# MLAB-project/radio-observer

Measured on AMD Instinct MI355X. Metric: FFT rows/sec (spectra/sec), N=32768 75% overlap, incl. per-row bolid scan, higher is better.
Workload: dtype f32; 1 GPU; C3/C4: synthetic IQ 48 kHz, FFT bins=32768, overlap=24576 (75%), Nuttall window, waterfall magnitude rows + BolidRecorder scan; input=float32 I/Q resident in HBM, output=float32 rows in HBM, parallelism=time-chunk per GPU

## Files before the change

### include/ro_stft.h

```cpp
#ifndef RO_STFT_H
#define RO_STFT_H

#include <stddef.h>
#include <stdint.h>

#ifdef __cplusplus
extern "C" {
#endif

#define RO_OK               0
#define RO_ERR_INVALID     (-1)
#define RO_ERR_UNSUPPORTED (-2)
#define RO_ERR_HIP         (-3)
#define RO_ERR_NOMEM       (-4)
#define RO_ERR_STATE       (-5)

#define RO_ABI_VERSION 5

enum { RO_WINDOW_NUTTALL = 0, RO_WINDOW_HANN = 1, RO_WINDOW_CUSTOM = 2 };

enum { RO_IQ_F32 = 0, RO_IQ_I16 = 1, RO_IQ_F64 = 2 };

enum { RO_PRECISION_F32 = 0, RO_PRECISION_F64 = 1 };

// ... 305 lines not shown
                               ro_unit_summary_t *d_unit_summary, void *stream);

int ro_snapshot_units_host(const ro_snapshot_t *dir, int64_t dir_capacity, const ro_snap_summary_t *snap_summary,
                           const float *arena, int64_t arena_floats, int32_t cols, const ro_band_window_t *slot_windows,
                           ro_fits_unit_t *unit_dir, void *units, int64_t units_bytes, ro_unit_summary_t *unit_summary);
int ro_raw_units_host(const ro_raw_capture_t *raw_dir, int64_t dir_capacity, const ro_raw_summary_t *raw_summary,
                      const float *arena, int64_t arena_floats,
                      ro_fits_unit_t *unit_dir, void *units, int64_t units_bytes, ro_unit_summary_t *unit_summary);

#define RO_MAX_PERIODIC 8
enum { RO_PERIODIC_WRITTEN = 0, RO_PERIODIC_LOST = 1, RO_PERIODIC_NO_ROOM = 2 };

typedef struct ro_periodic {
    int32_t          snapshot_rows;
    ro_band_window_t window;
} ro_periodic_t;

typedef struct ro_periodic_entry {
    int64_t index;
    int64_t first_row;
    int64_t due_row;
    int64_t offset;
    int64_t bytes;
    int32_t rows;
    int32_t naxis1;
    int32_t recorder;
    int32_t status;
} ro_periodic_entry_t;

typedef struct ro_periodic_summary {
    int64_t entries, written, lost, no_room;
    int64_t unlisted;
    int64_t units_bytes;
    int64_t needed_bytes;
    int64_t reserved;
} ro_periodic_summary_t;

int ro_snapshot_rows(int sample_rate, int bins, int overlap, int snapshot_length);

int ro_periodic_plan(const ro_periodic_t *recorders, int count, int64_t *next_index, int64_t head_row, int final,
                     int64_t ring_rows, int32_t cols, int64_t units_bytes,
                     ro_periodic_entry_t *dir, int64_t capacity, ro_periodic_summary_t *summary);

int ro_stft_periodic_units_resident(ro_stft_t *h, const ro_row_ring_t *ring, const ro_periodic_t *recorders, int count,
                                    const ro_periodic_entry_t *dir, int64_t entries, void *d_units, int64_t units_bytes,
                                    void *stream);

int ro_periodic_units_host(const ro_row_ring_t *ring, const ro_periodic_t *recorders, int count,
                           const ro_periodic_entry_t *dir, int64_t entries, void *units, int64_t units_bytes);

#define RO_LEVEL_BLOCK 720

typedef struct ro_level_range {
    float ln_min, ln_max;
} ro_level_range_t;

int ro_stft_snapshot_levels_resident(ro_stft_t *h, const ro_snapshot_t *d_dir, int64_t dir_capacity,
                                     const ro_snap_summary_t *d_snap_summary, const float *d_arena, int64_t arena_floats,
                                     int32_t cols, const ro_band_window_t *slot_windows,
                                     ro_fits_unit_t *d_level_dir, ro_level_range_t *d_ranges, void *d_levels,
                                     int64_t levels_bytes, ro_unit_summary_t *d_level_summary, void *stream);

int ro_stft_periodic_levels_resident(ro_stft_t *h, const ro_row_ring_t *ring, const ro_periodic_t *recorders, int count,
                                     const ro_periodic_entry_t *dir, int64_t entries, ro_level_range_t *d_ranges,
                                     void *d_levels, int64_t levels_bytes, void *stream);

int ro_snapshot_levels_host(const ro_snapshot_t *dir, int64_t dir_capacity, const ro_snap_summary_t *snap_summary,
                            const float *arena, int64_t arena_floats, int32_t cols, const ro_band_window_t *slot_windows,
                            ro_fits_unit_t *level_dir, ro_level_range_t *ranges, void *levels, int64_t levels_bytes,
                            ro_unit_summary_t *level_summary);
int ro_periodic_levels_host(const ro_row_ring_t *ring, const ro_periodic_t *recorders, int count,
                            const ro_periodic_entry_t *dir, int64_t entries, ro_level_range_t *ranges, void *levels,
                            int64_t levels_bytes);

#define RO_PNG_ALIGN 16

int64_t ro_png_bytes(int32_t naxis1, int64_t naxis2);

int ro_stft_levels_png_resident(ro_stft_t *h, const ro_fits_unit_t *d_level_dir, int64_t dir_capacity,
                                const ro_unit_summary_t *d_level_summary, const void *d_levels, int64_t levels_bytes,
                                ro_fits_unit_t *d_png_dir, void *d_png, int64_t png_bytes,
                                ro_unit_summary_t *d_png_summary, void *stream);

int ro_levels_png_host(const ro_fits_unit_t *level_dir, int64_t dir_capacity, const ro_unit_summary_t *level_summary,
                       const void *levels, int64_t levels_bytes, ro_fits_unit_t *png_dir, void *png, int64_t png_bytes,
                       ro_unit_summary_t *png_summary);

int ro_stft_levels_png_deflate_resident(ro_stft_t *h, const ro_fits_unit_t *d_level_dir, int64_t dir_capacity,
                                        const ro_unit_summary_t *d_level_summary, const void *d_levels, int64_t levels_bytes,
                                        ro_fits_unit_t *d_png_dir, void *d_png, int64_t png_bytes,
                                        ro_unit_summary_t *d_png_summary, void *stream);

int ro_levels_png_deflate_host(const ro_fits_unit_t *level_dir, int64_t dir_capacity, const ro_unit_summary_t *level_summary,
                               const void *levels, int64_t levels_bytes, ro_fits_unit_t *png_dir, void *png, int64_t png_bytes,
                               ro_unit_summary_t *png_summary);

int ro_periodic_level_dir(const ro_periodic_entry_t *dir, int64_t entries, ro_fits_unit_t *level_dir,
                          ro_unit_summary_t *level_summary);

typedef struct ro_resize_info {
    int64_t jobs;
    int64_t h_items, v_items;
    int64_t mid_bytes;
    int64_t plan_bytes;
    int64_t reserved[3];
} ro_resize_info_t;

int ro_resize_shape(int32_t naxis1, int64_t naxis2, int32_t width, int32_t *out_naxis1, int64_t *out_naxis2);

int ro_resize_plan(const ro_fits_unit_t *level_dir, int64_t dir_capacity, const ro_unit_summary_t *level_summary,
                   int64_t levels_bytes, int32_t width, ro_fits_unit_t *out_level_dir, int64_t out_levels_bytes,
                   ro_unit_summary_t *out_level_summary, void *plan, int64_t plan_bytes, ro_resize_info_t *info);

int ro_stft_levels_resize_resident(ro_stft_t *h, const ro_resize_info_t *info, const void *d_plan, const void *d_levels,
                                   int64_t levels_bytes, void *d_out_levels, int64_t out_levels_bytes, void *stream);

int ro_levels_resize_host(const ro_resize_info_t *info, const void *plan, const void *levels, int64_t levels_bytes,
                          void *out_levels, int64_t out_levels_bytes);

int ro_stft_time_resident(ro_stft_t *h, const void *d_iq, int format, int64_t samples,
                          int64_t first_row, int64_t rows,
                          float *d_rows, int64_t row_stride,
                          float *d_tile, ro_scan_record_t *d_records, void *stream,
                          int iters, float *ms_out, float *kernel_ms_out);

int ro_stft_push(ro_stft_t *h, const void *iq, int format, int64_t samples, int64_t *rows_ready);
int ro_stft_flush(ro_stft_t *h, int64_t *rows_ready);
int ro_stft_fetch(ro_stft_t *h, int64_t max_rows, int first_col, int cols,
                  float *rows_out, ro_scan_record_t *records_out,
                  int64_t *first_row_index, int64_t *rows_got);
int ro_stft_fetch_sets(ro_stft_t *h, int64_t max_rows, int first_col, int cols, float *rows_out,
                       ro_scan_record_t *records_out, ro_scan_record_t *extra_out,
                       int64_t *first_row_index, int64_t *rows_got);
int ro_stft_set_tile_windows(ro_stft_t *h, const ro_band_window_t *windows, int count);
int ro_stft_tile_windows(const ro_stft_t *h, ro_band_window_t *out );
int ro_stft_rows_complete(ro_stft_t *h, int64_t *rows);
int ro_stft_set_row_sink(ro_stft_t *h, float *base, int64_t row_stride, int64_t capacity_rows, int64_t first_slot);
void *ro_pinned_alloc(int device, size_t bytes);
void  ro_pinned_free(void *p);
int   ro_pinned_check(const void *p, size_t bytes);
int ro_stft_fetch_ln(ro_stft_t *h, int64_t max_rows, float *tile_out, float *ln_out, float *minmax_out,
                     ro_scan_record_t *records_out, int64_t *first_row_index, int64_t *rows_got);
int ro_stft_reset(ro_stft_t *h);
typedef struct ro_stft_timing {
    int64_t push_calls;  double push_ms_avg, push_ms_max;
    int64_t batches;     double batch_gpu_ms_avg, batch_gpu_ms_max;
    int64_t batch_rows;  double row_gpu_us_avg;
    int64_t fetch_calls; double fetch_ms_avg, fetch_ms_max;
} ro_stft_timing_t;
int ro_stft_timing(ro_stft_t *h, ro_stft_timing_t *out, int reset );
int ro_stft_stats(const ro_stft_t *h, int64_t *samples_in, int64_t *rows_out,
                  int64_t *launches, double *kernel_ms_total);

#ifdef __cplusplus
}
#endif
#endif
```

### radio-observer_amd/__init__.py

```python
from . import build as _build
from . import capi
from .capi import (
    Stft, StftError, Bands, BandWindow, ScanRecord, PinnedArray, library, library_path, hip_runtimes, require_one_hip_runtime,
    clamp_overlap, fft_sample_rate, frequency_to_bin, bin_to_frequency, time_to_fft_samples,
    row_count, window_table, bins_supported, device_count, shard_rows, shard_samples, shard_max_rows,
    stitch_rows, ln_levels, band_supported, bands_hull, band_windows_supported, bands_windows,
    tile_windows_supported, merge_windows, events_host, Detector,
    EVENT_DTYPE, DETECT_STATE_DTYPE, DETECT_SUMMARY_DTYPE,
    snapshots_host, RowRing, ROW_RING, SNAPSHOT_DTYPE, SNAP_SUMMARY_DTYPE, RO_SNAP_CAPTURED, RO_SNAP_EMPTY, RO_SNAP_LOST,
    raw_host, IqSpan, RAW_CAPTURE_DTYPE, RAW_SUMMARY_DTYPE, RO_MAX_IQ_SPANS,
    snapshot_units_host, raw_units_host, FITS_UNIT_DTYPE, UNIT_SUMMARY_DTYPE, RO_FITS_BLOCK,
    RO_UNIT_WRITTEN, RO_UNIT_SKIPPED, RO_UNIT_NO_ROOM, RO_UNIT_INVALID,
    snapshot_rows, periodic_plan, periodic_units_host, periodic_recorders, PERIODIC_DTYPE, PERIODIC_ENTRY_DTYPE,
    PERIODIC_SUMMARY_DTYPE, RO_MAX_PERIODIC, RO_PERIODIC_WRITTEN, RO_PERIODIC_LOST, RO_PERIODIC_NO_ROOM,
    snapshot_levels_host, periodic_levels_host, LEVEL_RANGE_DTYPE, RO_LEVEL_BLOCK,
    png_bytes, levels_png_host, levels_png_deflate_host, periodic_level_dir, RO_PNG_ALIGN,
    resize_shape, resize_plan, levels_resize_host, RESIZE_INFO_DTYPE,
    RO_WINDOW_NUTTALL, RO_WINDOW_HANN, RO_WINDOW_CUSTOM, RO_IQ_F32, RO_IQ_I16, RO_IQ_F64,
    RO_PRECISION_F32, RO_PRECISION_F64,
)

def sharding():
    import importlib
    return importlib.import_module(__name__ + ".timeshard")


__all__ = ["capi", "Stft", "StftError", "Bands", "ScanRecord", "library"]
```

### radio-observer_amd/build.py

```python
import os
import subprocess
import sys

HERE = os.path.dirname(os.path.abspath(__file__))
CSRC = os.path.join(HERE, "csrc")
LIB = os.path.join(HERE, "libro_stft.so")
SOURCES = ["ro_kernels.hip", "ro_stft32k.hip", "ro_fourstep.hip", "ro_f64reg.hip", "ro_band.hip", "ro_band_f64.hip", "ro_band_windows.hip", "ro_band_windows_f64.hip", "ro_scan_sets.hip", "ro_cut_windows.hip", "ro_events.hip", "ro_snapshots.hip", "ro_raw.hip", "ro_units.hip", "ro_periodic.hip", "ro_levels.hip", "ro_png.hip", "ro_png_deflate.hip", "ro_resize.hip", "ro_stft_capi.cpp", "ro_abi_helpers.cpp",
           "ro_exchange.cpp", "ro_stream.cpp", "ro_czt.cpp", "ro_snapshots.cpp", "ro_raw.cpp", "ro_units.cpp", "ro_periodic.cpp", "ro_levels.cpp", "ro_png.cpp", "ro_png_deflate.cpp", "ro_resize.cpp"]
HEADERS = ["ro_kernels.h", "ro_band.h", "ro_band_f64.h", "ro_band_windows.h", "ro_events.h", "ro_snapshots.h", "ro_raw.h", "ro_units.h", "ro_periodic.h", "ro_levels.h", "ro_png.h", "ro_png_deflate.h", "ro_resize.h", "ro_png_crc_device.h", "ro_pack_plan.h", "ro_host.h", "ro_owned.h", "ro_fft_device.h", "ro_fft_planar.h", "ro_k32_lds.h", "ro_device_util.h", "ro_f64_device.h", "ro_narrow.h", os.path.join("..", "..", "include", "ro_stft.h")]

HIPCC_FLAGS = ["-O3", "--offload-arch=gfx950", "-std=c++17", "-fno-slp-vectorize", "-fPIC", "-shared",
               "-Wall", "-Wno-unused-function", "-Wno-inline-asm"]


def _stale():
    if not os.path.exists(LIB):
        return True
    t = os.path.getmtime(LIB)
    deps = [os.path.join(CSRC, s) for s in SOURCES + HEADERS] + [os.path.abspath(__file__)]
    return any(os.path.getmtime(d) > t for d in deps)


def build(force=False, verbose=False):
    if not force and not _stale():
        return LIB
    hipcc = os.environ.get("HIPCC", "hipcc")
    cmd = [hipcc] + HIPCC_FLAGS + ["-o", LIB] + [os.path.join(CSRC, s) for s in SOURCES]
    if verbose:
        print(" ".join(cmd), file=sys.stderr)
    subprocess.check_call(cmd)
    return LIB


if __name__ == "__main__":
    build(force="--force" in sys.argv, verbose=True)
    print(LIB)
```

### radio-observer_amd/capi.py

```python
import ctypes as C
import os

import numpy as np

from . import build as _build

RO_WINDOW_NUTTALL, RO_WINDOW_HANN, RO_WINDOW_CUSTOM = 0, 1, 2
RO_IQ_F32, RO_IQ_I16, RO_IQ_F64 = 0, 1, 2
RO_PRECISION_F32, RO_PRECISION_F64 = 0, 1
RO_MAX_EXTRA_BANDS = 7
RO_MAX_BAND_WINDOWS = 8
RO_MAX_TILE_WINDOWS = 8

RO_OK = 0
_ERR_NAMES = {-1: "RO_ERR_INVALID", -2: "RO_ERR_UNSUPPORTED", -3: "RO_ERR_HIP", -4: "RO_ERR_NOMEM",
              -5: "RO_ERR_STATE"}


class StftError(RuntimeError):
    def __init__(self, code, text):
        super().__init__("%s (%d): %s" % (_ERR_NAMES.get(code, "RO_ERR"), code, text))
        self.code = code


class Bands(C.Structure):
    _fields_ = [("low_noise", C.c_int32), ("noise_width", C.c_int32), ("low_detect", C.c_int32),
                ("detect_width", C.c_int32), ("avg_bins", C.c_int32)]


class BandWindow(C.Structure):
    _fields_ = [("first_col", C.c_int32), ("cols", C.c_int32)]

    def __iter__(self):
        return iter((self.first_col, self.cols))

    def __repr__(self):
        return "BandWindow(%d, %d)" % (self.first_col, self.cols)


class ScanRecord(C.Structure):
    _fields_ = [("noise", C.c_float), ("peak", C.c_int32), ("average", C.c_float)]


class Timing(C.Structure):
    _fields_ = [("push_calls", C.c_int64), ("push_ms_avg", C.c_double), ("push_ms_max", C.c_double),
                ("batches", C.c_int64), ("batch_gpu_ms_avg", C.c_double), ("batch_gpu_ms_max", C.c_double),
                ("batch_rows", C.c_int64), ("row_gpu_us_avg", C.c_double),
                ("fetch_calls", C.c_int64), ("fetch_ms_avg", C.c_double), ("fetch_ms_max", C.c_double)]


SCAN_DTYPE = np.dtype([("noise", np.float32), ("peak", np.int32), ("average", np.float32)])


class Detector(C.Structure):
    _fields_ = [("advance", C.c_int32), ("jitter", C.c_int32)]


EVENT_DTYPE = np.dtype([("fire_row", np.int64), ("start_row", np.int64), ("length", np.int64), ("noise", np.float32),
                        ("peak", np.int32), ("magnitude", np.float32), ("reserved", np.int32)])
DETECT_STATE_DTYPE = np.dtype([("first_detect_row", np.int64), ("last_detect_row", np.int64), ("noise", np.float32),
                               ("peak", np.int32), ("magnitude", np.float32), ("open", np.int32)])
DETECT_SUMMARY_DTYPE = np.dtype([("events", np.int64), ("detect_rows", np.int64), ("marginal_rows", np.int64)])

RO_SNAP_CAPTURED, RO_SNAP_EMPTY, RO_SNAP_LOST = 0, 1, 2


class RowRing(C.Structure):
    _fields_ = [("d_rows", C.c_void_p), ("stride", C.c_int64), ("ring_rows", C.c_int64), ("cols", C.c_int32),
                ("reserved", C.c_int32)]


ROW_RING = RowRing
SNAPSHOT_DTYPE = np.dtype([("event", EVENT_DTYPE), ("first_row", np.int64), ("offset", np.int64), ("rows", np.int32),
                           ("slot", np.int32), ("status", np.int32), ("reserved", np.int32)])
SNAP_SUMMARY_DTYPE = np.dtype([("resolved", np.int64), ("captured", np.int64), ("empty", np.int64), ("lost", np.int64),
                               ("pending", np.int64), ("pending_dropped", np.int64), ("unlisted", np.int64),
                               ("arena_floats", np.int64)])


RO_MAX_IQ_SPANS = 4


class IqSpan(C.Structure):
    _fields_ = [("d_iq", C.c_void_p), ("first_sample", C.c_int64), ("samples", C.c_int64), ("format", C.c_int32),
                ("reserved", C.c_int32)]


RAW_CAPTURE_DTYPE = np.dtype([("event", EVENT_DTYPE), ("first_sample", np.int64), ("samples", np.int64), ("offset", np.int64),
                              ("slot", np.int32), ("status", np.int32)])
RAW_SUMMARY_DTYPE = np.dtype([("resolved", np.int64), ("captured", np.int64), ("empty", np.int64), ("lost", np.int64),
                              ("pending", np.int64), ("pending_dropped", np.int64), ("arena_floats", np.int64),
                              ("reserved", np.int64)])

RO_FITS_BLOCK = 2880
RO_UNIT_WRITTEN, RO_UNIT_SKIPPED, RO_UNIT_NO_ROOM, RO_UNIT_INVALID = 0, 1, 2, 3
FITS_UNIT_DTYPE = np.dtype([("offset", np.int64), ("bytes", np.int64), ("naxis2", np.int64), ("naxis1", np.int32),
                            ("status", np.int32)])
UNIT_SUMMARY_DTYPE = np.dtype([("entries", np.int64), ("written", np.int64), ("skipped", np.int64), ("no_room", np.int64),
                               ("invalid", np.int64), ("units_bytes", np.int64), ("needed_bytes", np.int64),
                               ("reserved", np.int64)])

RO_MAX_PERIODIC = 8
RO_PERIODIC_WRITTEN, RO_PERIODIC_LOST, RO_PERIODIC_NO_ROOM = 0, 1, 2
PERIODIC_DTYPE = np.dtype([("snapshot_rows", np.int32), ("first_col", np.int32), ("cols", np.int32)])
PERIODIC_ENTRY_DTYPE = np.dtype([("index", np.int64), ("first_row", np.int64), ("due_row", np.int64), ("offset", np.int64),
                                 ("bytes", np.int64), ("rows", np.int32), ("naxis1", np.int32), ("recorder", np.int32),
                                 ("status", np.int32)])
PERIODIC_SUMMARY_DTYPE = np.dtype([("entries", np.int64), ("written", np.int64), ("lost", np.int64), ("no_room", np.int64),
                                   ("unlisted", np.int64), ("units_bytes", np.int64), ("needed_bytes", np.int64),
                                   ("reserved", np.int64)])

RO_LEVEL_BLOCK = 720
LEVEL_RANGE_DTYPE = np.dtype([("ln_min", np.float32), ("ln_max", np.float32)])
RESIZE_INFO_DTYPE = np.dtype([("jobs", np.int64), ("h_items", np.int64), ("v_items", np.int64), ("mid_bytes", np.int64),
                              ("plan_bytes", np.int64), ("reserved", np.int64, (3,))])


class Config(C.Structure):
    _fields_ = [("struct_size", C.c_uint32), ("bins", C.c_int32), ("overlap", C.c_int32),
                ("sample_rate", C.c_int32), ("window_kind", C.c_int32),
                ("window_table", C.POINTER(C.c_float)), ("iq_gain", C.c_double),
                ("iq_phase_shift", C.c_int32), ("device", C.c_int32), ("max_batch_rows", C.c_int32),
                ("enable_scan", C.c_int32), ("bands", Bands), ("tile_first_col", C.c_int32),
                ("tile_cols", C.c_int32), ("spare_cus_per_xcd", C.c_int32), ("precision", C.c_int32),
                ("tile_ln", C.c_int32)]


_EXPORTS = {
    "ro_abi_version": (C.c_int, []),
    "ro_last_error": (C.c_char_p, []),
    "ro_device_count": (C.c_int, []),
    "ro_clamp_overlap": (C.c_int, [C.c_int, C.c_int]),
    "ro_fft_sample_rate": (C.c_float, [C.c_int, C.c_int, C.c_int]),
    "ro_frequency_to_bin": (C.c_int, [C.c_int, C.c_int, C.c_float]),
    "ro_bin_to_frequency": (C.c_float, [C.c_int, C.c_int, C.c_int]),
    "ro_time_to_fft_samples": (C.c_int, [C.c_double, C.c_float]),
    "ro_row_count": (C.c_int64, [C.c_int64, C.c_int, C.c_int]),
    "ro_window_table": (C.c_int, [C.c_int, C.c_int, C.POINTER(C.c_float)]),
    "ro_bins_supported": (C.c_int, [C.c_int]),
    "ro_shard_rows": (C.c_int, [C.c_int64, C.c_int, C.c_int, C.POINTER(C.c_int64), C.POINTER(C.c_int64)]),
    "ro_shard_samples": (C.c_int, [C.c_int64, C.c_int64, C.c_int, C.c_int, C.POINTER(C.c_int64),
                                   C.POINTER(C.c_int64)]),
    "ro_shard_max_rows": (C.c_int64, [C.c_int64, C.c_int]),
    "ro_stitch_rows": (C.c_int, [C.c_void_p, C.c_int64, C.c_int, C.c_size_t, C.c_void_p]),
    "ro_direct_schedule": (C.c_int, [C.c_int, C.c_int, C.c_int64, C.c_int, C.POINTER(C.c_int), C.POINTER(C.c_int),
                                     C.POINTER(C.c_int64), C.POINTER(C.c_int64)]),
    "ro_allgather_rows": (C.c_int, [C.c_void_p, C.c_void_p, C.c_int64, C.c_int64, C.c_int, C.c_int, C.c_size_t,
                                    C.c_void_p, C.c_void_p, C.c_void_p]),
    "ro_gather_rows": (C.c_int, [C.c_void_p, C.c_void_p, C.c_int64, C.c_int64, C.c_int, C.c_int, C.c_int, C.c_size_t,
                                 C.c_void_p, C.c_void_p]),
    "ro_allgather_rows_direct": (C.c_int, [C.c_void_p, C.c_void_p, C.c_int64, C.c_int64, C.c_int, C.c_int, C.c_size_t,
                                           C.c_void_p, C.c_void_p]),
    "ro_stitch_rows_device": (C.c_int, [C.c_void_p, C.c_int64, C.c_int, C.c_size_t, C.c_void_p, C.c_void_p]),
    "ro_stft_create": (C.c_int, [C.POINTER(Config), C.POINTER(C.c_void_p)]),
    "ro_stft_destroy": (C.c_int, [C.c_void_p]),
    "ro_stft_get_window": (C.c_int, [C.c_void_p, C.POINTER(C.c_float)]),
    "ro_stft_hop": (C.c_int, [C.c_void_p]),
    "ro_stft_bins": (C.c_int, [C.c_void_p]),
    "ro_stft_device_name": (C.c_int, [C.c_void_p, C.c_char_p, C.c_size_t]),
    "ro_stft_set_bands": (C.c_int, [C.c_void_p, C.POINTER(Bands)]),
    "ro_stft_set_extra_bands": (C.c_int, [C.c_void_p, C.POINTER(Bands), C.c_int]),
    "ro_stft_extra_bands": (C.c_int, [C.c_void_p, C.POINTER(Bands)]),
    "ro_stft_run_resident_sets": (C.c_int, [C.c_void_p, C.c_void_p, C.c_int, C.c_int64, C.c_int64, C.c_int64,
                                            C.c_void_p, C.c_int64, C.c_void_p, C.c_void_p, C.c_void_p, C.c_void_p]),
    "ro_stft_scan_sets_resident": (C.c_int, [C.c_void_p, C.c_void_p, C.c_int64, C.c_int64, C.c_void_p, C.c_void_p,
                                             C.c_void_p]),
    "ro_stft_fetch_sets": (C.c_int, [C.c_void_p, C.c_int64, C.c_int, C.c_int, C.POINTER(C.c_float),
                                     C.POINTER(ScanRecord), C.POINTER(ScanRecord), C.POINTER(C.c_int64),
                                     C.POINTER(C.c_int64)]),
    "ro_stft_run_resident": (C.c_int, [C.c_void_p, C.c_void_p, C.c_int, C.c_int64, C.c_int64, C.c_int64,
                                       C.c_void_p, C.c_int64, C.c_void_p, C.c_void_p, C.c_void_p]),
    "ro_stft_run_resident_ln": (C.c_int, [C.c_void_p, C.c_void_p, C.c_int, C.c_int64, C.c_int64, C.c_int64,
                                          C.c_void_p, C.c_int64, C.c_void_p, C.c_void_p, C.c_void_p, C.c_void_p,
                                          C.c_void_p]),
    "ro_ln_levels": (C.c_int, [C.c_void_p, C.c_int64, C.c_float, C.c_float, C.c_void_p]),
    "ro_stft_fetch_ln": (C.c_int, [C.c_void_p, C.c_int64, C.c_void_p, C.c_void_p, C.c_void_p, C.c_void_p,
                                   C.POINTER(C.c_int64), C.POINTER(C.c_int64)]),
    "ro_stft_spectra_resident": (C.c_int, [C.c_void_p, C.c_void_p, C.c_int, C.c_int64, C.c_int64, C.c_int64,
                                           C.c_void_p, C.c_int64, C.c_void_p]),
    "ro_stft_scan_resident": (C.c_int, [C.c_void_p, C.c_void_p, C.c_int64, C.c_int64, C.c_void_p,
                                        C.c_void_p]),
    "ro_stft_ln_tile_resident": (C.c_int, [C.c_void_p, C.c_void_p, C.c_int64, C.c_int64, C.c_int, C.c_int,
                                           C.c_void_p, C.c_void_p, C.c_void_p, C.c_void_p]),
    "ro_stft_band_supported": (C.c_int, [C.c_int, C.c_int]),
    "ro_stft_band_supported_precision": (C.c_int, [C.c_int, C.c_int, C.c_int]),
    "ro_bands_hull": (C.c_int, [C.POINTER(Bands), C.c_int, C.c_int, C.c_int, C.POINTER(C.c_int), C.POINTER(C.c_int)]),
    "ro_stft_band_resident": (C.c_int, [C.c_void_p, C.c_void_p, C.c_int, C.c_int64, C.c_int64, C.c_int64, C.c_int,
                                        C.c_int, C.c_void_p, C.c_int64, C.c_void_p, C.c_void_p]),
    "ro_stft_band_windows_supported": (C.c_int, [C.c_int, C.POINTER(BandWindow), C.c_int, C.c_int]),
    "ro_bands_windows": (C.c_int, [C.POINTER(Bands), C.c_int, C.c_int, C.c_int, C.c_int, C.POINTER(BandWindow),
                                   C.POINTER(C.c_int)]),
    "ro_stft_band_windows_resident": (C.c_int, [C.c_void_p, C.c_void_p, C.c_int, C.c_int64, C.c_int64, C.c_int64,
                                                C.POINTER(BandWindow), C.c_int, C.c_void_p, C.c_int64, C.c_void_p,
                                                C.c_void_p, C.c_void_p]),
    "ro_tile_windows_supported": (C.c_int, [C.c_int, C.POINTER(BandWindow), C.c_int]),
    "ro_merge_windows": (C.c_int, [C.POINTER(BandWindow), C.c_int, C.c_int, C.POINTER(BandWindow), C.POINTER(C.c_int),
                                   C.POINTER(C.c_int32)]),
    "ro_stft_cut_windows_resident": (C.c_int, [C.c_void_p, C.c_void_p, C.c_int64, C.c_int64, C.POINTER(BandWindow),
                                               C.c_int, C.c_void_p, C.c_int64, C.c_void_p]),
    "ro_stft_run_resident_windows": (C.c_int, [C.c_void_p, C.c_void_p, C.c_int, C.c_int64, C.c_int64, C.c_int64,
                                               C.c_void_p, C.c_int64, C.POINTER(BandWindow), C.c_int, C.c_void_p,
                                               C.c_int64, C.c_void_p, C.c_void_p, C.c_void_p]),
    "ro_stft_set_tile_windows": (C.c_int, [C.c_void_p, C.POINTER(BandWindow), C.c_int]),
    "ro_stft_tile_windows": (C.c_int, [C.c_void_p, C.POINTER(BandWindow)]),
    "ro_events_host": (C.c_int, [C.c_void_p, C.c_int64, C.c_int64, C.c_int64, C.POINTER(Detector), C.c_void_p, C.c_void_p,
                                 C.c_int64, C.c_void_p, C.c_void_p]),
    "ro_stft_events_resident": (C.c_int, [C.c_void_p, C.c_void_p, C.c_void_p, C.c_int64, C.c_int64, C.POINTER(Detector),
                                          C.c_void_p, C.c_void_p, C.c_int64, C.c_void_p, C.c_void_p, C.c_void_p]),
    "ro_stft_run_resident_events": (C.c_int, [C.c_void_p, C.c_void_p, C.c_int, C.c_int64, C.c_int64, C.c_int64, C.c_void_p,
                                              C.c_int64, C.c_void_p, C.c_void_p, C.c_void_p, C.POINTER(Detector),
                                              C.c_void_p, C.c_void_p, C.c_int64, C.c_void_p, C.c_void_p, C.c_void_p]),
    "ro_stft_ring_put_resident": (C.c_int, [C.c_void_p, C.c_void_p, C.c_int64, C.c_int64, C.c_int64, C.POINTER(RowRing),
                                            C.c_void_p]),
    "ro_stft_snapshots_resident": (C.c_int, [C.c_void_p, C.c_void_p, C.c_int64, C.c_void_p, C.c_uint32, C.POINTER(C.c_int32),
                                             C.POINTER(RowRing), C.c_int64, C.c_void_p, C.c_void_p, C.c_int64, C.c_void_p,
                                             C.c_void_p, C.c_int64, C.c_void_p, C.c_void_p]),
    "ro_snapshots_host": (C.c_int, [C.c_void_p, C.c_int64, C.c_void_p, C.c_uint32, C.POINTER(C.c_int32), C.POINTER(RowRing),
                                    C.c_int64, C.c_void_p, C.c_void_p, C.c_int64, C.c_void_p, C.c_void_p, C.c_int64,
                                    C.c_void_p]),
    "ro_stft_raw_resident": (C.c_int, [C.c_void_p, C.c_void_p, C.c_int64, C.c_void_p, C.POINTER(IqSpan), C.c_int, C.c_void_p,
                                       C.c_void_p, C.c_int64, C.c_void_p, C.c_void_p, C.c_int64, C.c_void_p, C.c_void_p]),
    "ro_raw_host": (C.c_int, [C.c_int, C.c_int, C.c_int, C.c_void_p, C.c_int64, C.c_void_p, C.POINTER(IqSpan), C.c_int,
                              C.c_void_p, C.c_void_p, C.c_int64, C.c_void_p, C.c_void_p, C.c_int64, C.c_void_p]),
    "ro_stft_snapshot_units_resident": (C.c_int, [C.c_void_p, C.c_void_p, C.c_int64, C.c_void_p, C.c_void_p, C.c_int64, C.c_int32,
                                                  C.POINTER(BandWindow), C.c_void_p, C.c_void_p, C.c_int64, C.c_void_p,
                                                  C.c_void_p]),
    "ro_stft_raw_units_resident": (C.c_int, [C.c_void_p, C.c_void_p, C.c_int64, C.c_void_p, C.c_void_p, C.c_int64, C.c_void_p,
                                             C.c_void_p, C.c_int64, C.c_void_p, C.c_void_p]),
    "ro_snapshot_units_host": (C.c_int, [C.c_void_p, C.c_int64, C.c_void_p, C.c_void_p, C.c_int64, C.c_int32,
                                         C.POINTER(BandWindow), C.c_void_p, C.c_void_p, C.c_int64, C.c_void_p]),
    "ro_raw_units_host": (C.c_int, [C.c_void_p, C.c_int64, C.c_void_p, C.c_void_p, C.c_int64, C.c_void_p, C.c_void_p, C.c_int64,
                                    C.c_void_p]),
    "ro_snapshot_rows": (C.c_int, [C.c_int, C.c_int, C.c_int, C.c_int]),
    "ro_periodic_plan": (C.c_int, [C.c_void_p, C.c_int, C.c_void_p, C.c_int64, C.c_int, C.c_int64, C.c_int32, C.c_int64,
                                   C.c_void_p, C.c_int64, C.c_void_p]),
    "ro_stft_periodic_units_resident": (C.c_int, [C.c_void_p, C.POINTER(RowRing), C.c_void_p, C.c_int, C.c_void_p, C.c_int64,
                                                  C.c_void_p, C.c_int64, C.c_void_p]),
    "ro_periodic_units_host": (C.c_int, [C.POINTER(RowRing), C.c_void_p, C.c_int, C.c_void_p, C.c_int64, C.c_void_p, C.c_int64]),
    "ro_stft_snapshot_levels_resident": (C.c_int, [C.c_void_p, C.c_void_p, C.c_int64, C.c_void_p, C.c_void_p, C.c_int64, C.c_int32,
                                                   C.POINTER(BandWindow), C.c_void_p, C.c_void_p, C.c_void_p, C.c_int64,
                                                   C.c_void_p, C.c_void_p]),
    "ro_snapshot_levels_host": (C.c_int, [C.c_void_p, C.c_int64, C.c_void_p, C.c_void_p, C.c_int64, C.c_int32,
                                          C.POINTER(BandWindow), C.c_void_p, C.c_void_p, C.c_void_p, C.c_int64, C.c_void_p]),
    "ro_stft_periodic_levels_resident": (C.c_int, [C.c_void_p, C.POINTER(RowRing), C.c_void_p, C.c_int, C.c_void_p, C.c_int64,
                                                   C.c_void_p, C.c_void_p, C.c_int64, C.c_void_p]),
    "ro_periodic_levels_host": (C.c_int, [C.POINTER(RowRing), C.c_void_p, C.c_int, C.c_void_p, C.c_int64, C.c_void_p, C.c_void_p,
                                          C.c_int64]),
    "ro_png_bytes": (C.c_int64, [C.c_int32, C.c_int64]),
    "ro_stft_levels_png_resident": (C.c_int, [C.c_void_p, C.c_void_p, C.c_int64, C.c_void_p, C.c_void_p, C.c_int64, C.c_void_p,
                                              C.c_void_p, C.c_int64, C.c_void_p, C.c_void_p]),
    "ro_levels_png_host": (C.c_int, [C.c_void_p, C.c_int64, C.c_void_p, C.c_void_p, C.c_int64, C.c_void_p, C.c_void_p, C.c_int64,
                                     C.c_void_p]),
    "ro_stft_levels_png_deflate_resident": (C.c_int, [C.c_void_p, C.c_void_p, C.c_int64, C.c_void_p, C.c_void_p, C.c_int64,
                                                      C.c_void_p, C.c_void_p, C.c_int64, C.c_void_p, C.c_void_p]),
    "ro_levels_png_deflate_host": (C.c_int, [C.c_void_p, C.c_int64, C.c_void_p, C.c_void_p, C.c_int64, C.c_void_p, C.c_void_p,
                                             C.c_int64, C.c_void_p]),
    "ro_periodic_level_dir": (C.c_int, [C.c_void_p, C.c_int64, C.c_void_p, C.c_void_p]),
    "ro_resize_shape": (C.c_int, [C.c_int32, C.c_int64, C.c_int32, C.POINTER(C.c_int32), C.POINTER(C.c_int64)]),
    "ro_resize_plan": (C.c_int, [C.c_void_p, C.c_int64, C.c_void_p, C.c_int64, C.c_int32, C.c_void_p, C.c_int64, C.c_void_p,
                                 C.c_void_p, C.c_int64, C.c_void_p]),
    "ro_stft_levels_resize_resident": (C.c_int, [C.c_void_p, C.c_void_p, C.c_void_p, C.c_void_p, C.c_int64, C.c_void_p, C.c_int64,
                                                 C.c_void_p]),
    "ro_levels_resize_host": (C.c_int, [C.c_void_p, C.c_void_p, C.c_void_p, C.c_int64, C.c_void_p, C.c_int64]),
    "ro_stft_time_resident": (C.c_int, [C.c_void_p, C.c_void_p, C.c_int, C.c_int64, C.c_int64, C.c_int64,
                                        C.c_void_p, C.c_int64, C.c_void_p, C.c_void_p, C.c_void_p,
                                        C.c_int, C.POINTER(C.c_float), C.POINTER(C.c_float)]),
    "ro_stft_push": (C.c_int, [C.c_void_p, C.c_void_p, C.c_int, C.c_int64, C.POINTER(C.c_int64)]),
    "ro_stft_flush": (C.c_int, [C.c_void_p, C.POINTER(C.c_int64)]),
    "ro_stft_fetch": (C.c_int, [C.c_void_p, C.c_int64, C.c_int, C.c_int, C.POINTER(C.c_float),
                                C.POINTER(ScanRecord), C.POINTER(C.c_int64), C.POINTER(C.c_int64)]),
    "ro_stft_reset": (C.c_int, [C.c_void_p]),
    "ro_stft_rows_complete": (C.c_int, [C.c_void_p, C.POINTER(C.c_int64)]),
    "ro_stft_set_row_sink": (C.c_int, [C.c_void_p, C.c_void_p, C.c_int64, C.c_int64, C.c_int64]),
    "ro_pinned_alloc": (C.c_void_p, [C.c_int, C.c_size_t]),
    "ro_pinned_free": (None, [C.c_void_p]),
    "ro_pinned_check": (C.c_int, [C.c_void_p, C.c_size_t]),
    "ro_stft_timing": (C.c_int, [C.c_void_p, C.c_void_p, C.c_int]),
    "ro_stft_stats": (C.c_int, [C.c_void_p, C.POINTER(C.c_int64), C.POINTER(C.c_int64),
                                C.POINTER(C.c_int64), C.POINTER(C.c_double)]),
}

_lib = None


def library_path():
    return _build.LIB


def exported_symbols():
    return sorted(_EXPORTS)


def hip_runtimes():
    found = set()
    try:
        with open("/proc/self/maps") as f:
            for line in f:
                path = line.rsplit(None, 1)[-1]
                if "libamdhip64" in os.path.basename(path):
                    found.add(os.path.realpath(path))
    except OSError:
        pass
    return sorted(found)


def require_one_hip_runtime():
    rts = hip_runtimes()
    if len(rts) > 1:
        raise StftError(-5, "two HIP runtimes are mapped into this process (%s): import torch BEFORE radio-observer_amd "
                            "loads libro_stft.so, so that both use the same one" % ", ".join(rts))


def library():
    global _lib
    if _lib is not None:
        return _lib
    path = os.environ.get("RO_STFT_LIB")
    if not path:
        path = _build.LIB
        if not os.path.exists(path):
            _build.build()
    lib = C.CDLL(path)
    for name, (res, args) in _EXPORTS.items():
        fn = getattr(lib, name)
        fn.restype = res
        fn.argtypes = args
    _lib = lib
    return lib


class PinnedArray:

    def __init__(self, rows, cols, device=0):
        n = rows * cols * 4
        self._p = library().ro_pinned_alloc(device, n)
        if not self._p:
            raise MemoryError("ro_pinned_alloc(%d bytes) failed" % n)
        self.array = np.ctypeslib.as_array((C.c_float * (rows * cols)).from_address(self._p)).reshape(rows, cols)

    def close(self):
        if self._p:
            self.array = None
            library().ro_pinned_free(self._p)
            self._p = None

    def __del__(self):
        try:
            self.close()
        except Exception:
            pass


def _check(rc):
    if rc != RO_OK:
        raise StftError(rc, (library().ro_last_error() or b"").decode("utf-8", "replace"))


def clamp_overlap(bins, overlap):
    return library().ro_clamp_overlap(bins, overlap)


def fft_sample_rate(sample_rate, bins, overlap):
    return library().ro_fft_sample_rate(sample_rate, bins, overlap)


def frequency_to_bin(bins, sample_rate, frequency):
    return library().ro_frequency_to_bin(bins, sample_rate, frequency)


def bin_to_frequency(bins, sample_rate, bin_):
    return library().ro_bin_to_frequency(bins, sample_rate, bin_)


def time_to_fft_samples(seconds, fft_rate):
    return library().ro_time_to_fft_samples(seconds, fft_rate)


def row_count(samples, bins, overlap):
    return int(library().ro_row_count(int(samples), bins, overlap))


def window_table(kind, bins):
    w = np.empty(bins, dtype=np.float32)
    _check(library().ro_window_table(kind, bins, w.ctypes.data_as(C.POINTER(C.c_float))))
    return w


def shard_rows(total_rows, world, rank):
    first, rows = C.c_int64(), C.c_int64()
    _check(library().ro_shard_rows(int(total_rows), world, rank, C.byref(first), C.byref(rows)))
    return first.value, rows.value


def shard_samples(first_row, rows, bins, overlap):
    s0, ns = C.c_int64(), C.c_int64()
    _check(library().ro_shard_samples(int(first_row), int(rows), bins, overlap, C.byref(s0), C.byref(ns)))
    return s0.value, ns.value


def shard_max_rows(total_rows, world):
    n = library().ro_shard_max_rows(int(total_rows), world)
    if n < 0:
        _check(int(n))
    return int(n)


def direct_schedule(world, rank, total_rows, k):
    to, frm = C.c_int(), C.c_int()
    f, n = C.c_int64(), C.c_int64()
    _check(library().ro_direct_schedule(world, rank, int(total_rows), k, C.byref(to), C.byref(frm), C.byref(f), C.byref(n)))
    return to.value, frm.value, f.value, n.value


def stitch_rows(gathered, total_rows, world):
    g = np.ascontiguousarray(gathered)
    row_bytes = g.strides[0]
    out = np.empty((int(total_rows),) + g.shape[1:], dtype=g.dtype)
    _check(library().ro_stitch_rows(C.c_void_p(g.ctypes.data), int(total_rows), world, row_bytes,
                                    C.c_void_p(out.ctypes.data)))
    return out


def ln_levels(ln, mn, mx):
    a = np.ascontiguousarray(ln, dtype=np.float32)
    out = np.empty(a.shape, np.uint8)
    _check(library().ro_ln_levels(C.c_void_p(a.ctypes.data), a.size, float(mn), float(mx), C.c_void_p(out.ctypes.data)))
    return out


def bins_supported(bins):
    return bool(library().ro_bins_supported(bins))

# ... 189 lines not shown

def periodic_plan(recorders, next_index, head_row, final, ring_rows, cols, units_bytes, capacity):
    recs = periodic_recorders(recorders)
    if not isinstance(next_index, np.ndarray) or next_index.dtype != np.int64 or next_index.ndim != 1 or \
            next_index.shape[0] < len(recs) or not next_index.flags.c_contiguous:
        raise ValueError("next_index: a C-contiguous int64 array [count]")
    directory = np.zeros(max(capacity, 1), PERIODIC_ENTRY_DTYPE)
    out = np.zeros(1, PERIODIC_SUMMARY_DTYPE)
    p = lambda a: C.c_void_p(a.ctypes.data)
    _check(library().ro_periodic_plan(p(recs) if len(recs) else None, len(recs), p(next_index), head_row, 1 if final else 0,
                                      ring_rows, cols, units_bytes, p(directory) if capacity > 0 else None, capacity, p(out)))
    return directory[:int(out["entries"][0])], out[0]


def periodic_units_host(ring, recorders, directory, units_bytes, cols=None):
    ring = np.asarray(ring)
    if ring.dtype != np.float32 or ring.ndim != 2 or not ring.flags.c_contiguous:
        raise ValueError("ring: a C-contiguous float32 array [ring_rows, stride]")
    desc = RowRing(ring.ctypes.data, ring.shape[1], ring.shape[0], ring.shape[1] if cols is None else cols, 0)
    recs = periodic_recorders(recorders)
    directory = np.ascontiguousarray(directory)
    if directory.dtype != PERIODIC_ENTRY_DTYPE or directory.ndim != 1:
        raise ValueError("directory: PERIODIC_ENTRY_DTYPE [entries]")
    units = np.zeros(max(units_bytes, 1), np.uint8)
    p = lambda a: C.c_void_p(a.ctypes.data)
    _check(library().ro_periodic_units_host(C.byref(desc), p(recs) if len(recs) else None, len(recs),
                                            p(directory) if len(directory) else None, len(directory),
                                            p(units) if units_bytes > 0 else None, units_bytes))
    written = directory[directory["status"] == RO_PERIODIC_WRITTEN]
    used = 0 if not len(written) else int(written[-1]["offset"]) + -(-int(written[-1]["bytes"]) // RO_FITS_BLOCK) * RO_FITS_BLOCK
    return units[:used]


def snapshot_levels_host(directory, snap_summary, arena, cols, slot_windows, levels_bytes):
    directory = np.ascontiguousarray(directory)
    if directory.dtype != SNAPSHOT_DTYPE or directory.ndim != 1 or snap_summary.itemsize != 64 or snap_summary.size < 1:
        raise ValueError("directory: SNAPSHOT_DTYPE [n] with the summary of the call that wrote them")
    arena = np.ascontiguousarray(arena)
    if arena.dtype != np.float32 or arena.ndim != 1:
        raise ValueError("arena: float32 [arena_floats]")
    dcap = directory.shape[0]
    level_dir = np.zeros(max(dcap, 1), FITS_UNIT_DTYPE)
    ranges = np.zeros(max(dcap, 1), LEVEL_RANGE_DTYPE)
    levels = np.zeros(max(levels_bytes, 1), np.uint8)
    out = np.zeros(1, UNIT_SUMMARY_DTYPE)
    p = lambda a: C.c_void_p(a.ctypes.data)
    _check(library().ro_snapshot_levels_host(p(directory) if dcap else None, dcap, p(snap_summary), p(arena) if arena.size else None,
                                             arena.size, cols, _slot_windows(slot_windows), p(level_dir), p(ranges),
                                             p(levels) if levels_bytes > 0 else None, levels_bytes, p(out)))
    n = int(out["entries"][0])
    return level_dir[:n], ranges[:n], levels[:int(out["units_bytes"][0])], out[0]


def periodic_levels_host(ring, recorders, directory, levels_bytes, cols=None):
    ring = np.asarray(ring)
    if ring.dtype != np.float32 or ring.ndim != 2 or not ring.flags.c_contiguous:
        raise ValueError("ring: a C-contiguous float32 array [ring_rows, stride]")
    desc = RowRing(ring.ctypes.data, ring.shape[1], ring.shape[0], ring.shape[1] if cols is None else cols, 0)
    recs = periodic_recorders(recorders)
    directory = np.ascontiguousarray(directory)
    if directory.dtype != PERIODIC_ENTRY_DTYPE or directory.ndim != 1:
        raise ValueError("directory: PERIODIC_ENTRY_DTYPE [entries]")
    ranges = np.zeros(max(len(directory), 1), LEVEL_RANGE_DTYPE)
    levels = np.zeros(max(levels_bytes, 1), np.uint8)
    p = lambda a: C.c_void_p(a.ctypes.data)
    _check(library().ro_periodic_levels_host(C.byref(desc), p(recs) if len(recs) else None, len(recs),
                                             p(directory) if len(directory) else None, len(directory), p(ranges),
                                             p(levels) if levels_bytes > 0 else None, levels_bytes))
    written = directory[directory["status"] == RO_PERIODIC_WRITTEN]
    used = 0 if not len(written) else (int(written[-1]["offset"]) + -(-int(written[-1]["bytes"]) // RO_FITS_BLOCK) * RO_FITS_BLOCK) // 4
    return ranges[:len(directory)], levels[:used]


RO_PNG_ALIGN = 16


def png_bytes(naxis1, naxis2):
    n = int(library().ro_png_bytes(int(naxis1), int(naxis2)))
    if n < 0:
        _check(n)
    return n


def _levels_png_host(call, level_dir, level_summary, levels, png_room, dir_capacity):
    level_dir = np.ascontiguousarray(level_dir)
    level_summary = np.ascontiguousarray(level_summary).reshape(-1)
    if level_dir.dtype != FITS_UNIT_DTYPE or level_dir.ndim != 1 or level_summary.dtype != UNIT_SUMMARY_DTYPE or level_summary.size < 1:
        raise ValueError("level_dir: FITS_UNIT_DTYPE [n] with the UNIT_SUMMARY_DTYPE of the call that wrote them")
    levels = np.ascontiguousarray(levels)
    if levels.dtype != np.uint8 or levels.ndim != 1:
        raise ValueError("levels: uint8 [levels_bytes]")
    dcap = level_dir.shape[0] if dir_capacity is None else dir_capacity
    png_dir = np.zeros(max(dcap, 1), FITS_UNIT_DTYPE)
    png = np.zeros(max(png_room, 1), np.uint8)
    out = np.zeros(1, UNIT_SUMMARY_DTYPE)
    p = lambda a: C.c_void_p(a.ctypes.data)
    _check(call(p(level_dir) if dcap else None, dcap, p(level_summary), p(levels) if levels.size else None,
                levels.size, p(png_dir), p(png) if png_room > 0 else None, png_room, p(out)))
    return png_dir[:int(out["entries"][0])], png[:int(out["units_bytes"][0])], out[0]


def levels_png_host(level_dir, level_summary, levels, png_room, dir_capacity=None):
    return _levels_png_host(library().ro_levels_png_host, level_dir, level_summary, levels, png_room, dir_capacity)


def levels_png_deflate_host(level_dir, level_summary, levels, png_room, dir_capacity=None):
    return _levels_png_host(library().ro_levels_png_deflate_host, level_dir, level_summary, levels, png_room, dir_capacity)


def periodic_level_dir(directory):
    directory = np.ascontiguousarray(directory)
    if directory.dtype != PERIODIC_ENTRY_DTYPE or directory.ndim != 1:
        raise ValueError("directory: PERIODIC_ENTRY_DTYPE [entries]")
    level_dir = np.zeros(max(len(directory), 1), FITS_UNIT_DTYPE)
    out = np.zeros(1, UNIT_SUMMARY_DTYPE)
    p = lambda a: C.c_void_p(a.ctypes.data)
    _check(library().ro_periodic_level_dir(p(directory) if len(directory) else None, len(directory), p(level_dir), p(out)))
    return level_dir[:len(directory)], out[0]


def resize_shape(naxis1, naxis2, width):
    w, h = C.c_int32(), C.c_int64()
    _check(library().ro_resize_shape(int(naxis1), int(naxis2), int(width), C.byref(w), C.byref(h)))
    return w.value, h.value


def resize_plan(level_dir, level_summary, levels_bytes, width, out_levels_bytes, dir_capacity=None):
    level_dir = np.ascontiguousarray(level_dir)
    level_summary = np.ascontiguousarray(level_summary).reshape(-1)
    if level_dir.dtype != FITS_UNIT_DTYPE or level_dir.ndim != 1 or level_summary.dtype != UNIT_SUMMARY_DTYPE or level_summary.size < 1:
        raise ValueError("level_dir: FITS_UNIT_DTYPE [n] with the UNIT_SUMMARY_DTYPE of the call that wrote them")
    dcap = level_dir.shape[0] if dir_capacity is None else dir_capacity
    out_dir = np.zeros(max(dcap, 1), FITS_UNIT_DTYPE)
    out = np.zeros(1, UNIT_SUMMARY_DTYPE)
    info = np.zeros(1, RESIZE_INFO_DTYPE)
    p = lambda a: C.c_void_p(a.ctypes.data)
    args = (p(level_dir) if dcap else None, dcap, p(level_summary), int(levels_bytes), int(width), p(out_dir), int(out_levels_bytes), p(out))
    _check(library().ro_resize_plan(*args, None, 0, p(info)))
    plan = np.zeros(int(info["plan_bytes"][0]) // 8, np.int64).view(np.uint8)
    _check(library().ro_resize_plan(*args, p(plan), plan.size, p(info)))
    return out_dir[:int(out["entries"][0])], out[0], plan, info


def levels_resize_host(info, plan, levels, out_levels_bytes):
    info = np.ascontiguousarray(info).reshape(-1)
    plan, levels = np.ascontiguousarray(plan), np.ascontiguousarray(levels)
    if info.dtype != RESIZE_INFO_DTYPE or info.size < 1 or plan.dtype != np.uint8 or levels.dtype != np.uint8 or levels.ndim != 1:
        raise ValueError("info: RESIZE_INFO_DTYPE; plan, levels: uint8")
    out = np.zeros(max(out_levels_bytes, 1), np.uint8)
    p = lambda a: C.c_void_p(a.ctypes.data)
    _check(library().ro_levels_resize_host(p(info), p(plan), p(levels) if levels.size else None, levels.size,
                                           p(out) if out_levels_bytes > 0 else None, out_levels_bytes))
    return out[:out_levels_bytes]


def device_count():
    n = library().ro_device_count()
    if n < 0:
        _check(n)
    return n


def _ptr(x):
    if x is None:
        return None
    if hasattr(x, "data_ptr"):
        return C.c_void_p(x.data_ptr())
    return C.c_void_p(int(x))


class Stft:

    def __init__(self, bins=32768, overlap=0, sample_rate=48000, window=RO_WINDOW_NUTTALL,
                 window_table=None, iq_gain=0.0, iq_phase_shift=0, device=0, max_batch_rows=0,
                 bands=None, tile=None, spare_cus_per_xcd=0, precision=RO_PRECISION_F32, tile_ln=False,
                 extra_bands=None):
        cfg = Config()
        cfg.struct_size = C.sizeof(Config)
        cfg.bins, cfg.overlap, cfg.sample_rate = bins, overlap, sample_rate
        cfg.window_kind = window
        self._wt = None
        if window_table is not None:
            self._wt = np.ascontiguousarray(window_table, dtype=np.float32)
            if self._wt.size != bins:
                raise ValueError("window_table must have `bins` entries")
            cfg.window_kind = RO_WINDOW_CUSTOM
            cfg.window_table = self._wt.ctypes.data_as(C.POINTER(C.c_float))
        cfg.iq_gain = iq_gain
        cfg.iq_phase_shift = iq_phase_shift
        cfg.device = device
        cfg.max_batch_rows = max_batch_rows
        if bands is not None:
            cfg.enable_scan = 1
            cfg.bands = bands
        if tile is not None:
            cfg.tile_first_col, cfg.tile_cols = tile
        cfg.spare_cus_per_xcd = spare_cus_per_xcd
        cfg.precision = precision
        cfg.tile_ln = 1 if tile_ln else 0
        self._h = C.c_void_p()
        lib = library()
        require_one_hip_runtime()
        _check(lib.ro_stft_create(C.byref(cfg), C.byref(self._h)))
        self.bins = bins
        self.hop = library().ro_stft_hop(self._h)
        self.scan_enabled = bands is not None
        self.tile = tile
        self.extra_count = 0
        self.image_cols = 0
        if extra_bands:
            try:
                self.set_extra_bands(extra_bands)
            except Exception:
                self.close()
                raise

    def close(self):
        if getattr(self, "_h", None) and self._h.value:
            library().ro_stft_destroy(self._h)
            self._h = C.c_void_p()

    def __del__(self):
        try:
            self.close()
        except Exception:
            pass

    def __enter__(self):
        return self

    def __exit__(self, *exc):
        self.close()

    @property
    def window(self):
        w = np.empty(self.bins, dtype=np.float32)
        _check(library().ro_stft_get_window(self._h, w.ctypes.data_as(C.POINTER(C.c_float))))
        return w

    @property
    def device_name(self):
        buf = C.create_string_buffer(256)
        _check(library().ro_stft_device_name(self._h, buf, 256))
        return buf.value.decode()

    def set_bands(self, bands):
        _check(library().ro_stft_set_bands(self._h, C.byref(bands)))
        self.scan_enabled = True

    def set_extra_bands(self, sets):
        sets = list(sets or [])
        arr = (Bands * max(len(sets), 1))(*sets)
        _check(library().ro_stft_set_extra_bands(self._h, arr, len(sets)))
        self.extra_count = len(sets)

    @property
    def extra_bands(self):
        arr = (Bands * RO_MAX_EXTRA_BANDS)()
        n = library().ro_stft_extra_bands(self._h, arr)
        if n < 0:
            _check(n)
        return [arr[i] for i in range(n)]

    def run_resident_sets(self, d_iq, fmt, samples, first_row, rows, d_rows, row_stride=None, d_tile=None,
                          d_records=None, d_extra=None, stream=None):
        _check(library().ro_stft_run_resident_sets(self._h, _ptr(d_iq), fmt, samples, first_row, rows,
                                                   _ptr(d_rows), row_stride or self.bins, _ptr(d_tile),
                                                   _ptr(d_records), _ptr(d_extra), _ptr(stream)))

    def events_resident(self, rows, detectors, d_state, d_records=None, d_extra=None, first_row=0, d_events=None,
                        capacity=0, d_summary=None, d_detect=None, stream=None):
        if len(detectors) != 1 + self.extra_count:
            raise ValueError("detectors: one per slot, %d" % (1 + self.extra_count))
        _check(library().ro_stft_events_resident(self._h, _ptr(d_records), _ptr(d_extra), first_row, rows,
                                                 _detectors(detectors), _ptr(d_state), _ptr(d_events), capacity,
                                                 _ptr(d_summary), _ptr(d_detect), _ptr(stream)))

    def run_resident_events(self, d_iq, fmt, samples, first_row, rows, d_rows, detectors, d_state, row_stride=None,
                            d_tile=None, d_records=None, d_extra=None, d_events=None, capacity=0, d_summary=None,
                            d_detect=None, stream=None):
        if len(detectors) != 1 + self.extra_count:
            raise ValueError("detectors: one per slot, %d" % (1 + self.extra_count))
        _check(library().ro_stft_run_resident_events(self._h, _ptr(d_iq), fmt, samples, first_row, rows, _ptr(d_rows),
                                                     row_stride or self.bins, _ptr(d_tile), _ptr(d_records),
                                                     _ptr(d_extra), _detectors(detectors), _ptr(d_state), _ptr(d_events),
                                                     capacity, _ptr(d_summary), _ptr(d_detect), _ptr(stream)))

    def ring_put_resident(self, d_image, first_row, rows, ring, image_stride=None, stream=None):
        _check(library().ro_stft_ring_put_resident(self._h, _ptr(d_image), ring.cols if image_stride is None else image_stride,
                                                   first_row, rows, C.byref(ring), _ptr(stream)))

    def snapshots_resident(self, slot_mask, snapshot_rows, ring, head_row, d_pending, d_pending_count, pending_capacity,
                           d_dir, d_arena, arena_floats, d_snap_summary, d_events=None, capacity=0, d_summary=None,
                           stream=None):
        rows_arr, _ = _snapshot_rows(snapshot_rows, slot_mask)
        _check(library().ro_stft_snapshots_resident(self._h, _ptr(d_events), capacity, _ptr(d_summary), slot_mask, rows_arr,
                                                    C.byref(ring), head_row, _ptr(d_pending), _ptr(d_pending_count),
                                                    pending_capacity, _ptr(d_dir), _ptr(d_arena), arena_floats,
                                                    _ptr(d_snap_summary), _ptr(stream)))

    def raw_resident(self, d_dir, dir_capacity, d_snap_summary, spans, d_pending, d_pending_count, pending_capacity,
                     d_raw_dir, d_arena, arena_floats, d_raw_summary, stream=None):
        arr, count = _spans(spans)
        _check(library().ro_stft_raw_resident(self._h, _ptr(d_dir), dir_capacity, _ptr(d_snap_summary), arr, count,
                                              _ptr(d_pending), _ptr(d_pending_count), pending_capacity, _ptr(d_raw_dir),
                                              _ptr(d_arena), arena_floats, _ptr(d_raw_summary), _ptr(stream)))
# ... 88 lines not shown

    def spectra_resident(self, d_iq, fmt, samples, first_row, rows, d_spectra, stride=None, stream=None):
        _check(library().ro_stft_spectra_resident(self._h, _ptr(d_iq), fmt, samples, first_row, rows,
                                                  _ptr(d_spectra), stride or self.bins, _ptr(stream)))

    def band_resident(self, d_iq, fmt, samples, first_row, rows, first_col, cols, d_band, band_stride=None,
                      d_records=None, stream=None):
        _check(library().ro_stft_band_resident(self._h, _ptr(d_iq), fmt, samples, first_row, rows, first_col, cols,
                                               _ptr(d_band), band_stride or cols, _ptr(d_records), _ptr(stream)))

    def band_windows_resident(self, d_iq, fmt, samples, first_row, rows, windows, d_band, band_stride=None,
                              d_records=None, d_extra=None, stream=None):
        arr, n = _windows(windows)
        total = sum(arr[i].cols for i in range(n))
        _check(library().ro_stft_band_windows_resident(self._h, _ptr(d_iq), fmt, samples, first_row, rows, arr, n,
                                                       _ptr(d_band), band_stride or total, _ptr(d_records),
                                                       _ptr(d_extra), _ptr(stream)))

    def cut_windows_resident(self, d_rows, rows, windows, d_image, row_stride=None, image_stride=None, stream=None):
        arr, n = _windows(windows)
        total = sum(arr[i].cols for i in range(n))
        _check(library().ro_stft_cut_windows_resident(self._h, _ptr(d_rows), row_stride or self.bins, rows, arr, n,
                                                      _ptr(d_image), image_stride or total, _ptr(stream)))

    def run_resident_windows(self, d_iq, fmt, samples, first_row, rows, d_rows, windows, d_image, row_stride=None,
                             image_stride=None, d_records=None, d_extra=None, stream=None):
        arr, n = _windows(windows)
        total = sum(arr[i].cols for i in range(n))
        _check(library().ro_stft_run_resident_windows(self._h, _ptr(d_iq), fmt, samples, first_row, rows, _ptr(d_rows),
                                                      row_stride or self.bins, arr, n, _ptr(d_image),
                                                      image_stride or total, _ptr(d_records), _ptr(d_extra),
                                                      _ptr(stream)))

    def scan_resident(self, d_rows, rows, d_records, row_stride=None, stream=None):
        _check(library().ro_stft_scan_resident(self._h, _ptr(d_rows), row_stride or self.bins, rows,
                                               _ptr(d_records), _ptr(stream)))

    def ln_tile_resident(self, d_rows, rows, first_col, cols, d_ln=None, d_u8=None, d_minmax=None,
                         row_stride=None, stream=None):
        _check(library().ro_stft_ln_tile_resident(self._h, _ptr(d_rows), row_stride or self.bins, rows, first_col,
                                                  cols, _ptr(d_ln), _ptr(d_u8), _ptr(d_minmax), _ptr(stream)))

    def time_resident(self, d_iq, fmt, samples, first_row, rows, d_rows, iters, row_stride=None,
                      d_tile=None, d_records=None, stream=None):
        ms = (C.c_float * iters)()
        kern = (C.c_float * 2)()
        _check(library().ro_stft_time_resident(self._h, _ptr(d_iq), fmt, samples, first_row, rows,
                                               _ptr(d_rows), row_stride or self.bins, _ptr(d_tile),
                                               _ptr(d_records), _ptr(stream), iters, ms, kern))
        return np.array(ms[:], dtype=np.float64), float(kern[0]), float(kern[1])

    def push(self, iq):
        a = np.ascontiguousarray(iq)
        if a.dtype == np.complex64:
            a, fmt = a.view(np.float32), RO_IQ_F32
        elif a.dtype == np.complex128:
            a, fmt = a.view(np.float64), RO_IQ_F64
        elif a.dtype == np.float32:
            fmt = RO_IQ_F32
        elif a.dtype == np.float64:
            fmt = RO_IQ_F64
        elif a.dtype == np.int16:
            fmt = RO_IQ_I16
        else:
            raise TypeError("unsupported sample dtype %s" % a.dtype)
        n = a.size // 2
        ready = C.c_int64()
        _check(library().ro_stft_push(self._h, C.c_void_p(a.ctypes.data), fmt, n, C.byref(ready)))
        return ready.value

    def flush(self):
        ready = C.c_int64()
        _check(library().ro_stft_flush(self._h, C.byref(ready)))
        return ready.value

    def set_tile_windows(self, windows):
        arr, n = _windows(windows or [])
        _check(library().ro_stft_set_tile_windows(self._h, arr, n))
        self.image_cols = sum(arr[i].cols for i in range(n))

    @property
    def tile_windows(self):
        arr = (BandWindow * RO_MAX_TILE_WINDOWS)()
        n = library().ro_stft_tile_windows(self._h, arr)
        if n < 0:
            _check(n)
        return [BandWindow(arr[i].first_col, arr[i].cols) for i in range(n)]

    def _default_columns(self, first_col, cols):
        lo, n = (0, self.image_cols) if self.image_cols else self.tile if self.tile else (0, self.bins)
        if first_col is None:
            first_col = lo
        if cols is None:
            cols = lo + n - first_col
        return first_col, cols

    def fetch(self, max_rows, first_col=None, cols=None, want_records=None):
        first_col, cols = self._default_columns(first_col, cols)
        want_records = self.scan_enabled if want_records is None else want_records
        rows = np.empty((max_rows, cols), dtype=np.float32)
        recs = np.empty(max_rows, dtype=SCAN_DTYPE) if want_records else None
        first = C.c_int64()
        got = C.c_int64()
        _check(library().ro_stft_fetch(
            self._h, max_rows, first_col, cols, rows.ctypes.data_as(C.POINTER(C.c_float)),
            recs.ctypes.data_as(C.POINTER(ScanRecord)) if recs is not None else None,
            C.byref(first), C.byref(got)))
        g = got.value
        return first.value, rows[:g], (recs[:g] if recs is not None else None)

    def fetch_sets(self, max_rows, first_col=None, cols=None, want_rows=None, want_extra=True):
        first_col, cols = self._default_columns(first_col, cols)
        want_rows = (getattr(self, "_sink", None) is None) if want_rows is None else want_rows
        rows = np.empty((max_rows, cols), dtype=np.float32) if want_rows else None
        recs = np.empty(max_rows, dtype=SCAN_DTYPE) if self.scan_enabled else None
        count = self.extra_count
        extra = np.empty((max_rows, max(count, 1)), dtype=SCAN_DTYPE) if want_extra else None
        first, got = C.c_int64(), C.c_int64()
        _check(library().ro_stft_fetch_sets(
            self._h, max_rows, first_col if want_rows else 0, cols if want_rows else 0,
            rows.ctypes.data_as(C.POINTER(C.c_float)) if rows is not None else None,
            recs.ctypes.data_as(C.POINTER(ScanRecord)) if recs is not None else None,
            extra.ctypes.data_as(C.POINTER(ScanRecord)) if extra is not None else None,
            C.byref(first), C.byref(got)))
        g = got.value
        return (first.value, rows[:g] if rows is not None else None, recs[:g] if recs is not None else None,
                extra[:g, :count] if extra is not None else None)

    def reset(self):
        _check(library().ro_stft_reset(self._h))

    def set_row_sink(self, ring, first_slot=0):
        if ring is None:
            _check(library().ro_stft_set_row_sink(self._h, None, 0, 0, 0))
            self._sink = None
            return
        assert ring.dtype == np.float32 and ring.ndim == 2 and ring.flags["C_CONTIGUOUS"]
        _check(library().ro_stft_set_row_sink(self._h, C.c_void_p(ring.ctypes.data), ring.shape[1], ring.shape[0], first_slot))
        self._sink = ring

    def fetch_records(self, max_rows):
        recs = np.empty(max_rows, dtype=SCAN_DTYPE) if self.scan_enabled else None
        first, got = C.c_int64(), C.c_int64()
        _check(library().ro_stft_fetch(self._h, max_rows, 0, 0, None,
                                       recs.ctypes.data_as(C.POINTER(ScanRecord)) if recs is not None else None,
                                       C.byref(first), C.byref(got)))
        return first.value, got.value, (recs[:got.value] if recs is not None else None)

    def timing(self, reset=False):
        t = Timing()
        _check(library().ro_stft_timing(self._h, C.byref(t), 1 if reset else 0))
        return {k: getattr(t, k) for k, _ in Timing._fields_}

    def rows_complete(self):
        n = C.c_int64()
        _check(library().ro_stft_rows_complete(self._h, C.byref(n)))
        return n.value

    def stats(self):
        s, r, l = C.c_int64(), C.c_int64(), C.c_int64()
        ms = C.c_double()
        _check(library().ro_stft_stats(self._h, C.byref(s), C.byref(r), C.byref(l), C.byref(ms)))
        return {"samples_in": s.value, "rows_out": r.value, "launches": l.value,
                "kernel_ms_total": ms.value}
```

### radio-observer_amd/csrc/ro_host.h

```cpp
#pragma once

#include <hip/hip_runtime.h>

#include <dlfcn.h>

#include <algorithm>
#include <cmath>
#include <complex>
#include <cstdarg>
#include <cstdio>
#include <cstdlib>
#include <cstring>
#include <ctime>
#include <deque>
#include <string>
#include <mutex>
#include <vector>

#include "../../include/ro_stft.h"
#include "ro_kernels.h"
#include "ro_band.h"
#include "ro_band_f64.h"
#include "ro_band_windows.h"
#include "ro_events.h"
#include "ro_snapshots.h"
#include "ro_raw.h"
#include "ro_units.h"
#include "ro_periodic.h"
#include "ro_levels.h"
#include "ro_png.h"
#include "ro_png_deflate.h"
#include "ro_resize.h"
#include "ro_narrow.h"
#include "ro_owned.h"

#if defined(RO_DIAG) && !defined(RO_DIAG_KNOBS)
#define RO_DIAG_KNOBS 1
#endif

#ifndef RO_SPEC_SCRATCH_MB
#define RO_SPEC_SCRATCH_MB 2048
#endif
#ifndef RO_FOUR_SCRATCH_MB
#define RO_FOUR_SCRATCH_MB 1024
#endif
#ifndef RO_F64_SCRATCH_MB
#define RO_F64_SCRATCH_MB 128
#endif
#ifndef RO_F64_RING_ROWS
#define RO_F64_RING_ROWS 4
#endif
#ifndef RO_F64_WGS_PER_CU
#define RO_F64_WGS_PER_CU 1
#endif
#ifndef RO_STREAM_SLOTS
#define RO_STREAM_SLOTS 3
#endif
#ifndef RO_STREAM_GRAPH
#define RO_STREAM_GRAPH 1
#endif
#ifndef RO_GRAPH_TIME_EVERY
#define RO_GRAPH_TIME_EVERY 8
#endif

namespace ro {
namespace host {

int fail(int code, const char *fmt, ...) __attribute__((format(printf, 2, 3)));
const char *last_error_text();

#define HIP_TRY(expr)                                                                     \
    do {                                                                                  \
        hipError_t e_ = (expr);                                                           \
        if (e_ != hipSuccess)                                                             \
            return fail(RO_ERR_HIP, "%s failed: %s", #expr, hipGetErrorString(e_));       \
    } while (0)

inline double now_ms()
{
    timespec ts;
    clock_gettime(CLOCK_MONOTONIC, &ts);
    return ts.tv_sec * 1e3 + ts.tv_nsec * 1e-6;
}

struct Batch {
    int64_t first_row = 0;
    int64_t rows = 0;
    PinnedBlock<float> data;
    PinnedBlock<float> ln;
    PinnedBlock<float> minmax;
    PinnedBlock<ro_scan_record_t> records;
    PinnedBlock<ro_scan_record_t> extra;
    int64_t capacity_rows = 0;
    int64_t consumed = 0;
    hipEvent_t done = nullptr;
    hipEvent_t k0 = nullptr, k1 = nullptr;
    bool pending = false;
    bool timed = true;
};

template <typename T>
struct BandState {
    DeviceBlock<T> tw;
    DeviceBlock<T> t1;
    DeviceBlock<T> t2;
    DeviceBlock<int32_t> kcell;
    DeviceBlock<T> part;
    size_t part_bytes = 0;
};

}
}

struct ro_stft {
    template <typename T> using DeviceBlock = ro::host::DeviceBlock<T>;
    template <typename T> using PinnedBlock = ro::host::PinnedBlock<T>;

    ro_stft_config_t cfg{};
    int bins = 0, overlap = 0, hop = 0;
    int device = 0;
    std::string device_name;
    std::vector<float> window;
    DeviceBlock<float> d_window;
    DeviceBlock<float> d_window_k;
    DeviceBlock<float> d_window_k32;
    DeviceBlock<float2> d_twiddles;
    DeviceBlock<float4> d_twiddles_k;
    hipStream_t stream = nullptr;
    ro_bands_t extra[RO_MAX_EXTRA_BANDS] = {};
    int        extra_count = 0;
    ro_band_window_t tile_win[RO_MAX_TILE_WINDOWS] = {};
    int        tile_win_count = 0, tile_win_total = 0;

    int batch_rows = 0;
    int stage_fmt = RO_IQ_F32;
    bool stage_fmt_set = false;
    size_t  staged_have = 0;
    int64_t stream_sample0 = 0;
    float  *sink = nullptr;
    int64_t sink_stride = 0, sink_cap = 0, sink_first = 0;
    struct Slot {
        DeviceBlock<char> d_iq;
        DeviceBlock<float> d_rows;
        DeviceBlock<float> d_tile;
        DeviceBlock<float> d_ln;
        DeviceBlock<float> d_minmax;
        DeviceBlock<ro_scan_record_t> d_records;
        DeviceBlock<ro_scan_record_t> d_extra;
        DeviceBlock<float> d_image;
        PinnedBlock<char> h_in;
        hipEvent_t uploaded = nullptr;
        hipEvent_t staging_free = nullptr;
        hipEvent_t computed = nullptr;
        hipEvent_t drained = nullptr;
        hipStream_t    gstream = nullptr;
        hipGraphExec_t gexec = nullptr;
        int            graph_fmt = -1;
        int64_t        uses = 0;
        bool           on_gstream = false;
    } slot[RO_STREAM_SLOTS];
    bool slots_ready = false;
    hipStream_t s_in = nullptr, s_out = nullptr;
    bool graph_refused = false;
    int out_first = 0, out_cols = 0;
    int64_t batch_seq = 0;
    std::vector<ro::host::Batch *> batch_pool;
    int64_t rows_emitted = 0;
    std::deque<ro::host::Batch *> ready;
    int64_t rows_ready = 0;
    int64_t stat_samples = 0, stat_rows = 0, stat_launches = 0;
    double stat_kernel_ms = 0.0;
    ro_stft_timing_t timing{};
    double push_ms_sum = 0.0, batch_ms_sum = 0.0, fetch_ms_sum = 0.0;
    int64_t timed_batches = 0, timed_rows = 0;
    double  last_batch_ms = 0.0;
    int64_t graph_batches = 0;
    int     diag_time_every = 0, diag_done_only = 0, diag_direct = 0;
    hipEvent_t ev0 = nullptr, ev1 = nullptr;
    DeviceBlock<unsigned long long> d_stamps;

    DeviceBlock<unsigned> d_ln_keys;
    unsigned ln_calls = 0;
    bool    big = false;
    int     sub_bins = 0, dec = 0;
    DeviceBlock<float2> d_tw_combine;
    bool    dif = false;
    DeviceBlock<float>  d_window_dif;
    DeviceBlock<float2> d_dif_tw;
    DeviceBlock<float2> d_dif_shift;
    DeviceBlock<float2> d_spec;
    DeviceBlock<float>  d_ones;
    int64_t spec_rows = 0;
    DeviceBlock<float2> d_spec2;
    bool    four = false;
    DeviceBlock<float>  d_four_window;
    DeviceBlock<float2> d_four_tw_a, d_four_tw_b, d_four_tw_r;
    DeviceBlock<float>  d_four_z;
    int64_t four_rows = 0;
    bool    czt = false;
    int     czt_m = 0;
    ro_stft *inner = nullptr;
    DeviceBlock<float2> d_cw;
    DeviceBlock<float2> d_bc;
    DeviceBlock<float2> d_czt_a, d_czt_A;
    DeviceBlock<float>  d_czt_mag;
    int64_t czt_rows = 0;

    DeviceBlock<float> d_ln_part;
    int64_t ln_part_rows = 0;

    DeviceBlock<char> d_events_scratch;
    DeviceBlock<char> d_snap_scratch;
    DeviceBlock<char> d_raw_scratch;
    DeviceBlock<char> d_units_scratch[2];
    DeviceBlock<char> d_levels_scratch[2];
    DeviceBlock<char> d_png_scratch;
    DeviceBlock<char> d_png_deflate_scratch;
    DeviceBlock<char> d_resize_scratch;
    int cus = 0;

    std::vector<ro_band_window_t> band_key;
    ro::host::BandState<float2>  band;
    ro::host::BandState<double2> band64;

    bool     f64 = false;
    DeviceBlock<double2> d_tw_f64;
    bool     f64reg = false;
    DeviceBlock<float>   d_f64r_window;
    DeviceBlock<double2> d_f64r_tw[4];
    DeviceBlock<double2> d_scratch_d[2];
    int64_t  scratch_rows_d = 0;
    DeviceBlock<double2>  d_f64_ring;
    DeviceBlock<unsigned> d_f64_ctl;
    PinnedBlock<unsigned> h_f64_err;
    int       f64_ring_rows = 0, f64_wgs_per_cu = 0;
};

namespace ro {
namespace host {

void build_window(int kind, int bins, float *w);
const char *tile_windows_fault(int bins, const ro_band_window_t *w, int count, int64_t *total, int *which);
int tile_windows_check(const char *who, int bins, const ro_band_window_t *w, int count, int64_t *total);
ro::CutArgs make_cut_args(const ro_band_window_t *w, int count, float *d_image, int64_t image_stride);

ro::StftArgs make_stft_args(const ro_stft *h, const void *d_iq, int64_t first_row, int64_t rows, float *d_rows,
                            int64_t row_stride, float *d_tile = nullptr, ro_scan_record_t *d_records = nullptr,
                            float *d_ln = nullptr);
int launch_transform(ro_stft *h, const void *d_iq, int format, int64_t first_row, int64_t rows, float *d_rows,
                     int64_t row_stride, hipStream_t s, float *d_tile = nullptr, ro_scan_record_t *d_records = nullptr,
                     float *d_ln = nullptr);
int launch_tile_and_scan(ro_stft *h, const float *d_rows, int64_t row_stride, int64_t rows, float *d_tile,
                         ro_scan_record_t *d_records, hipStream_t s, float *d_ln = nullptr, float *d_minmax = nullptr,
                         ro_scan_record_t *d_extra = nullptr, const ro::CutArgs *cut = nullptr);
int check_bands(const ro_stft *h, const ro_bands_t &b);
int ensure_ln_part(ro_stft *h, int64_t rows);
int grow_scratch(DeviceBlock<char> &block, size_t need);
int device_cus(ro_stft *h, int *cus);
int scratch_for(ro_stft *h, DeviceBlock<char> &block, size_t need, int *cus);
int launch_spectra_big(ro_stft *h, const void *d_iq, int format, int64_t first_row, int64_t rows, float2 *d_out,
                       int64_t out_stride, hipStream_t s);

int ring_check(const char *who, const ro_row_ring_t *ring);

int png_check(const char *who, const char *d, bool aligned, const ro_fits_unit_t *level_dir, int64_t dir_capacity,
              const ro_unit_summary_t *level_summary, const void *levels, int64_t levels_bytes, const ro_fits_unit_t *png_dir,
              const void *png, int64_t png_bytes, const ro_unit_summary_t *png_summary);
void png_fill_args(ro::PngArgs &a, const ro_fits_unit_t *level_dir, int64_t dir_capacity, const ro_unit_summary_t *level_summary,
                   const void *levels, int64_t levels_bytes, ro_fits_unit_t *png_dir, void *png, int64_t png_bytes,
                   ro_unit_summary_t *png_summary);

struct DeflateCode {
    int64_t bytes;
    bool huffman;
    uint8_t length[ro::DEFLATE_SYMS];
    uint16_t reversed[ro::DEFLATE_SYMS];
};
DeflateCode deflate_code(const unsigned char *raw, int64_t len, bool last);
int64_t deflate_write_block(const unsigned char *raw, int64_t len, bool last, const DeflateCode *code, unsigned char *out);

struct UnitNames {
    const char *dir, *buf, *bytes, *summary;
};
int units_check(const char *who, const char *d, const UnitNames &names, bool raw, bool aligned, const void *dir,
                int64_t dir_capacity, const void *summary, const float *arena, int64_t arena_floats, int32_t cols,
                const ro_band_window_t *slot_windows, const ro_fits_unit_t *unit_dir, const void *units, int64_t units_bytes,
                const ro_unit_summary_t *unit_summary);
struct WalkWant {
    int32_t status;
    int32_t naxis1;
    int64_t naxis2;
    int64_t bytes;
    int64_t room;
};
template <class Want, class Emit>
void pack_walk(int64_t n, Want want, Emit emit, ro_fits_unit_t *dir, void *buf, int64_t buf_bytes, ro_unit_summary_t *summary)
{
    ro_unit_summary_t sum{};
    sum.entries = n;
    int64_t first = 0;
    for (int64_t d = 0; d < n; ++d) {
        const WalkWant w = want(d);
        ro_fits_unit_t out{};
        out.status = w.status;
        if (w.status == RO_UNIT_SKIPPED) sum.skipped += 1;
        else if (w.status == RO_UNIT_INVALID) sum.invalid += 1;
        else {
            out.bytes = w.bytes;
            out.naxis2 = w.naxis2;
            out.naxis1 = w.naxis1;
            if (first + w.room <= buf_bytes) {
                out.offset = first;
                unsigned char *dst = static_cast<unsigned char *>(buf) + first;
                emit(d, dst);
                std::memset(dst + w.bytes, 0, (size_t)(w.room - w.bytes));
                sum.written += 1;
                sum.units_bytes = first + w.room;
            } else {
                out.status = RO_UNIT_NO_ROOM;
                sum.no_room += 1;
            }
            first += w.room;
        }
        dir[d] = out;
    }
    sum.needed_bytes = first;
    *summary = sum;
}
inline WalkWant walk_want(const ro::UnitWant &w, int64_t elem, int64_t block)
{
    if (w.status != RO_UNIT_WRITTEN) return WalkWant{w.status, 0, 0, 0, 0};
    return WalkWant{w.status, w.naxis1, w.naxis2, elem * (int64_t)w.naxis1 * w.naxis2, ro::unit_blocks(w.naxis1, w.naxis2) * block};
}
inline int64_t entries_of(int64_t resolved, int64_t dir_capacity) { return std::min(std::max<int64_t>(resolved, 0), dir_capacity); }
inline ro::UnitWant unit_want_snapshot(const ro_snapshot_t &e, int32_t cols, int64_t arena_floats, const ro_band_window_t *slot_windows)
{
    const bool slot_ok = e.slot >= 0 && e.slot < ro::UNIT_SLOTS;
    return ro::unit_want_image(e.status, e.slot, e.rows, e.offset, cols, arena_floats, slot_ok ? slot_windows[e.slot].first_col : 0,
                               slot_ok ? slot_windows[e.slot].cols : 0);
}
void units_fill_args(ro::UnitsArgs &a, const void *dir, int64_t dir_capacity, const void *summary, const float *arena,
                     int64_t arena_floats, int32_t cols, const ro_band_window_t *slot_windows, ro_fits_unit_t *unit_dir,
                     void *units, int64_t units_bytes, ro_unit_summary_t *unit_summary);

struct PeriodicNames {
    const char *buf, *bytes, *room;
};
int periodic_check(const char *who, const char *d, const PeriodicNames &names, int64_t block, bool aligned,
                   const ro_row_ring_t *ring, const ro_periodic_t *recorders, int count, const ro_periodic_entry_t *dir,
                   int64_t entries, void *buf, int64_t buf_bytes, ro::PeriodicArgs *a);

int czt_length(int bins);
int czt_setup(ro_stft *h);
int launch_transform_czt(ro_stft *h, const void *d_iq, int format, int64_t first_row, int64_t rows, float *d_rows,
                         int64_t row_stride, hipStream_t s);

void destroy_batch(Batch *b);
void free_stream_slots(ro_stft *h);

}
}
```

### radio-observer_amd/csrc/ro_stft_capi.cpp

```cpp
#include "ro_host.h"

using namespace ro::host;

namespace {

std::vector<float2> build_twiddles(int bins)
{
    int radix[4];
    std::vector<float2> tw;
    if (!ro::stft_radices(bins, radix)) return tw;
    const long double two_pi = 8.0L * atanl(1.0L);
    long ns = radix[0];
    for (int s = 1; s < 4; ++s) {
        const int R = radix[s];
        if (R <= 1) continue;
        for (int r = 1; r < R; ++r)
            for (long k = 0; k < ns; ++k) {
                const long double ang = -two_pi * (long double)((long long)r * k) / (long double)(ns * R);
                tw.push_back(make_float2((float)cosl(ang), (float)sinl(ang)));
            }
        ns *= R;
    }
    return tw;
}
// ... 510 lines not shown

    {
        int xccs = 0;
        if (hipDeviceGetAttribute(&xccs, hipDeviceAttributeNumberOfXccs, cfg->device) == hipSuccess) {
            static bool said = false;
            if (xccs > 0 && xccs != 8 && !said) {
                said = true;
                fprintf(stderr, "libro_stft: device %d reports %d XCDs; the kernels' row placement is laid out for 8 (an MI355X in "
                                "SPX mode): rows are unaffected, the L2 sharing between neighbouring rows is lost\n", cfg->device, xccs);
            }
        } else {
            (void)hipGetLastError();
        }
    }

    h->window.resize(h->bins);
    if (cfg->window_kind == RO_WINDOW_CUSTOM)
        std::memcpy(h->window.data(), cfg->window_table, sizeof(float) * h->bins);
    else
        build_window(cfg->window_kind, h->bins, h->window.data());
    h->big = ro::big_supported(h->bins);
    h->f64 = cfg->precision != RO_PRECISION_F32;
    h->czt_m = czt_length(h->bins);
    h->czt = h->czt_m > 0;
    if (h->big && !h->f64) {
        const int sub = 32768, dec = h->bins / sub;
        bool four = ro::fourstep_supported(h->bins);
#ifdef RO_DIAG_KNOBS
        if (const char *e = getenv("RO_BIG_FORM")) four = std::strcmp(e, "dif") != 0 && four;
#endif
        h->four = four;
        h->dif = !four;
        h->sub_bins = sub;
        h->dec = dec;
    }
    const int plan_bins = h->czt ? 0 : h->big ? h->sub_bins : h->bins;
    std::vector<float2> tw = plan_bins ? build_twiddles(plan_bins) : std::vector<float2>();
    if (plan_bins && (int)tw.size() != ro::stft_twiddle_count(plan_bins)) {
        delete h;
        return fail(RO_ERR_STATE, "internal: twiddle table size mismatch");
    }

#define CREATE_TRY(expr)                                                                   \
    do {                                                                                   \
        hipError_t e2_ = (expr);                                                           \
        if (e2_ != hipSuccess) {                                                           \
            int rc2_ = fail(RO_ERR_HIP, "%s failed: %s", #expr, hipGetErrorString(e2_));   \
            ro_stft_destroy(h);                                                            \
            return rc2_;                                                                   \
        }                                                                                  \
    } while (0)
    CREATE_TRY(hipStreamCreateWithFlags(&h->stream, hipStreamNonBlocking));
    CREATE_TRY(hipEventCreate(&h->ev0));
    CREATE_TRY(hipEventCreate(&h->ev1));
    CREATE_TRY(h->d_window.upload(h->window));
    CREATE_TRY(h->d_ln_keys.alloc(16 * 2));
    if (tw.empty()) CREATE_TRY(h->d_twiddles.alloc(1));
    else CREATE_TRY(h->d_twiddles.upload(tw));
    if (!h->big && !h->czt) {
        std::vector<float> wk((size_t)h->bins);
        if (!ro::stft_window_layout(h->bins, h->window.data(), wk.data())) {
            ro_stft_destroy(h);
            return fail(RO_ERR_UNSUPPORTED, "no window layout for bins=%d", h->bins);
        }
        CREATE_TRY(h->d_window_k.upload(wk));
        if (h->bins == 32768) {
            ro::stft32k_window_layout(h->window.data(), wk.data());
            CREATE_TRY(h->d_window_k32.upload(wk));
        }
    }
    if (plan_bins) {
        const int units = ro::stft_packed_twiddle_count(plan_bins);
        std::vector<float4> pk((size_t)std::max(units, 1));
        if (units > 0) ro::stft_pack_twiddles(plan_bins, tw.data(), pk.data());
        CREATE_TRY(h->d_twiddles_k.upload(pk));
    }
    if (h->f64) {
        std::vector<double2> full = build_full_twiddles_f64(h->bins);
        CREATE_TRY(h->d_tw_f64.upload(full));
        h->f64reg = ro::f64reg_supported(h->bins);
#ifdef RO_DIAG
        if (const char *e = getenv("RO_F64_HBM")) h->f64reg = h->f64reg && atoi(e) == 0;
#endif
        if (h->f64reg) {
            ro::F64RegTables t;
            ro::f64reg_tables(h->bins, h->window.data(), t);
            CREATE_TRY(h->d_f64r_window.upload(t.window_k));
            const std::vector<double2> *tabs[4] = {&t.tw0, &t.tw1, &t.tw2, &t.tw3};
            for (int i = 0; i < 4; ++i)
                if (!tabs[i]->empty()) CREATE_TRY(h->d_f64r_tw[i].upload(*tabs[i]));
        }
    }
    if (h->big && h->dec > 1) {
        std::vector<float2> tc((size_t)h->bins);
        const long double two_pi = 8.0L * atanl(1.0L);
        for (int r = 0; r < h->dec; ++r)
            for (int k = 0; k < h->sub_bins; ++k) {
                const long double ang = -two_pi * (long double)((long long)r * k) / (long double)h->bins;
                tc[(size_t)r * h->sub_bins + k] = make_float2((float)cosl(ang), (float)sinl(ang));
            }
        CREATE_TRY(h->d_tw_combine.upload(tc));
    }
    if (h->big && h->dec > 1) {
        std::vector<float> ones((size_t)h->sub_bins, 1.0f);
        CREATE_TRY(h->d_ones.upload(ones));
    }
    if (h->dif) {
        std::vector<float> wk((size_t)h->bins);
        for (int r = 0; r < h->dec; ++r)
            if (!ro::stft_window_layout(h->sub_bins, h->window.data() + (size_t)r * h->sub_bins,
                                        wk.data() + (size_t)r * h->sub_bins)) {
                ro_stft_destroy(h);
                return fail(RO_ERR_UNSUPPORTED, "no window layout for bins=%d", h->sub_bins);
            }
        CREATE_TRY(h->d_window_dif.upload(wk));
        std::vector<float2> td((size_t)h->dec);
        const long double two_pi = 8.0L * atanl(1.0L);
        for (int j = 0; j < h->dec; ++j) {
            const long double ang = -two_pi * (long double)j / (long double)h->dec;
            long double c = cosl(ang), sn = sinl(ang);
            if ((4 * j) % h->dec == 0) { c = roundl(c); sn = roundl(sn); }
            td[(size_t)j] = make_float2((float)c, (float)sn);
        }
        CREATE_TRY(h->d_dif_tw.upload(td));
        std::vector<float2> ts((size_t)h->dec * 16, make_float2(1.0f, 0.0f));
        const long double span[3] = {32.0L, 1024.0L, 32768.0L};
        for (int q = 0; q < h->dec; ++q)
            for (int st = 0; st < 3; ++st)
                for (int i = 0; i < 5; ++i) {
                    const long double ang = -two_pi * ((long double)q / (long double)h->dec) * (long double)(1 << i) / span[st];
                    ts[(size_t)q * 16 + st * 5 + i] = make_float2((float)cosl(ang), (float)sinl(ang));
                }
        CREATE_TRY(h->d_dif_shift.upload(ts));
    }
    if (h->four) {
        std::vector<float> wa;
        std::vector<float2> ta, tb, tr;
        ro::fourstep_tables(h->bins, h->window.data(), wa, ta, tb, tr);
        CREATE_TRY(h->d_four_window.upload(wa));
        CREATE_TRY(h->d_four_tw_a.upload(ta));
        CREATE_TRY(h->d_four_tw_b.upload(tb));
        CREATE_TRY(h->d_four_tw_r.upload(tr));
    }
    if (h->czt) {
        const int rc = czt_setup(h);
        if (rc != RO_OK) { ro_stft_destroy(h); return rc; }
    }
#undef CREATE_TRY

    h->out_first = cfg->tile_cols > 0 ? cfg->tile_first_col : 0;
    h->out_cols = cfg->tile_cols > 0 ? cfg->tile_cols : h->bins;
    h->batch_rows = cfg->max_batch_rows > 0 ? cfg->max_batch_rows
                                            : std::max(1, (64 << 20) / (h->bins * 4));
#ifdef RO_DIAG_KNOBS
    if (const char *e = getenv("RO_GRAPH_TIME_EVERY")) h->diag_time_every = atoi(e);
    if (const char *e = getenv("RO_GRAPH_TWO_EVENTS")) h->diag_done_only = atoi(e) == 0;
    if (const char *e = getenv("RO_GRAPH_DIRECT")) h->diag_direct = atoi(e);
#endif
    *out = h;
    return RO_OK;
}

extern "C" int ro_stft_destroy(ro_stft_t *h)
{
    if (!h) return RO_OK;
    (void)hipSetDevice(h->device);
    if (h->s_in) (void)hipStreamSynchronize(h->s_in);
    if (h->stream) (void)hipStreamSynchronize(h->stream);
    if (h->s_out) (void)hipStreamSynchronize(h->s_out);
    for (ro_stft::Slot &sl : h->slot)
        if (sl.gstream) (void)hipStreamSynchronize(sl.gstream);
    free_stream_slots(h);
    while (!h->ready.empty()) {
        destroy_batch(h->ready.front());
        h->ready.pop_front();
    }
    for (Batch *b : h->batch_pool) destroy_batch(b);
    if (h->inner) (void)ro_stft_destroy(h->inner);
    if (h->ev0) (void)hipEventDestroy(h->ev0);
    if (h->ev1) (void)hipEventDestroy(h->ev1);
    if (h->stream) (void)hipStreamDestroy(h->stream);
    delete h;
    return RO_OK;
}

#ifdef RO_DIAG
extern "C" int ro_stft_debug_stamps(ro_stft_t *h, unsigned long long *out, int max_words)
{
    if (!h) return fail(RO_ERR_INVALID, "null handle");
    const int words = 4096 * 16;
    if (!h->d_stamps) {
        HIP_TRY(hipSetDevice(h->device));
        HIP_TRY(h->d_stamps.alloc(words));
        HIP_TRY(hipMemset(h->d_stamps, 0, sizeof(unsigned long long) * words));
        return RO_OK;
    }
    if (out) {
        HIP_TRY(hipDeviceSynchronize());
        HIP_TRY(hipMemcpy(out, h->d_stamps, sizeof(unsigned long long) * std::min(words, max_words),
                          hipMemcpyDeviceToHost));
    }
    return RO_OK;
}
#endif

extern "C" int ro_stft_get_window(const ro_stft_t *h, float *out)
{
    if (!h || !out) return fail(RO_ERR_INVALID, "null argument");
    std::memcpy(out, h->window.data(), sizeof(float) * h->bins);
    return RO_OK;
}

extern "C" int ro_stft_hop(const ro_stft_t *h) { return h ? h->hop : fail(RO_ERR_INVALID, "null handle"); }
extern "C" int ro_stft_bins(const ro_stft_t *h) { return h ? h->bins : fail(RO_ERR_INVALID, "null handle"); }

extern "C" int ro_stft_device_name(const ro_stft_t *h, char *buf, size_t len)
{
    if (!h || !buf || len == 0) return fail(RO_ERR_INVALID, "null argument");
    std::snprintf(buf, len, "%s", h->device_name.c_str());
    return RO_OK;
}

extern "C" int ro_stft_set_bands(ro_stft_t *h, const ro_bands_t *bands)
{
    if (!h || !bands) return fail(RO_ERR_INVALID, "null argument");
    int rc = check_bands(h, *bands);
    if (rc != RO_OK) return rc;
    h->cfg.bands = *bands;
    h->cfg.enable_scan = 1;
    return RO_OK;
}

static int run_resident(ro_stft_t *h, const void *d_iq, int format, int64_t samples, int64_t first_row, int64_t rows,
                        float *d_rows, int64_t row_stride, float *d_tile, ro_scan_record_t *d_records,
                        ro_scan_record_t *d_extra, void *stream, float *d_ln = nullptr, float *d_minmax = nullptr,
                        const ro::CutArgs *cut = nullptr)
{
    int rc = validate_resident(h, d_iq, format, samples, first_row, rows, d_rows, row_stride, d_tile,
                               d_records);
    if (rc != RO_OK) return rc;
    if (d_extra && h->extra_count == 0)
        return fail(RO_ERR_STATE, "extra records requested but no extra band sets are set (ro_stft_set_extra_bands)");
    if (rows == 0) return rc;
    HIP_TRY(hipSetDevice(h->device));
    hipStream_t s = (hipStream_t)stream;
    rc = launch_transform(h, d_iq, format, first_row, rows, d_rows, row_stride, s, d_tile, d_records, d_ln);
    if (rc != RO_OK) return rc;
    rc = launch_tile_and_scan(h, d_rows, row_stride, rows, d_tile, d_records, s, d_ln, d_minmax, d_extra, cut);
    if (rc != RO_OK) return rc;
    h->stat_launches += 1;
    h->stat_rows += rows;
    return RO_OK;
}

extern "C" int ro_stft_run_resident(ro_stft_t *h, const void *d_iq, int format, int64_t samples,
                                    int64_t first_row, int64_t rows, float *d_rows, int64_t row_stride,
                                    float *d_tile, ro_scan_record_t *d_records, void *stream)
{
    return run_resident(h, d_iq, format, samples, first_row, rows, d_rows, row_stride, d_tile, d_records, nullptr, stream);
}

extern "C" int ro_stft_run_resident_sets(ro_stft_t *h, const void *d_iq, int format, int64_t samples, int64_t first_row,
                                         int64_t rows, float *d_rows, int64_t row_stride, float *d_tile,
                                         ro_scan_record_t *d_records, ro_scan_record_t *d_extra, void *stream)
{
    return run_resident(h, d_iq, format, samples, first_row, rows, d_rows, row_stride, d_tile, d_records, d_extra, stream);
}

extern "C" int ro_stft_run_resident_ln(ro_stft_t *h, const void *d_iq, int format, int64_t samples, int64_t first_row,
                                       int64_t rows, float *d_rows, int64_t row_stride, float *d_tile, float *d_ln_tile,
                                       float *d_ln_minmax, ro_scan_record_t *d_records, void *stream)
{
    int rc = validate_resident(h, d_iq, format, samples, first_row, rows, d_rows, row_stride, d_tile, d_records);
    if (rc != RO_OK || rows == 0) return rc;
    if (!h->cfg.tile_ln) return fail(RO_ERR_STATE, "this handle was not created with tile_ln");
    if (!d_tile) return fail(RO_ERR_INVALID, "the log image is cut from the tile: d_tile is required");
    if (d_ln_minmax && !d_ln_tile) return fail(RO_ERR_INVALID, "the range comes with the log image: pass d_ln_tile too");
    return run_resident(h, d_iq, format, samples, first_row, rows, d_rows, row_stride, d_tile, d_records, nullptr, stream,
                        d_ln_tile, d_ln_minmax);
}

extern "C" int ro_stft_spectra_resident(ro_stft_t *h, const void *d_iq, int format, int64_t samples,
                                        int64_t first_row, int64_t rows, float *d_spectra, int64_t stride,
                                        void *stream)
{
    int rc = validate_resident(h, d_iq, format, samples, first_row, rows, d_spectra, stride, nullptr, nullptr);
    if (rc != RO_OK) return rc;
    if (h->czt) return fail(RO_ERR_UNSUPPORTED, "complex spectra are available for power-of-two bins");
    HIP_TRY(hipSetDevice(h->device));
    if (h->f64) {
        if (!h->f64reg)
            return fail(RO_ERR_UNSUPPORTED, "complex spectra of RO_PRECISION_F64 handles are available up to 65536 bins");
        ro::F64RegArgs r = make_f64reg_args(h, d_iq, first_row, rows, d_spectra, stride);
        r.spectra = 1;
        HIP_TRY(ro::launch_f64reg(h->bins, format, r, (hipStream_t)stream));
        return RO_OK;
    }
    if (h->big)
        return launch_spectra_big(h, d_iq, format, first_row, rows, reinterpret_cast<float2 *>(d_spectra), stride,
                                  (hipStream_t)stream);
    ro::StftArgs a = make_stft_args(h, d_iq, first_row, rows, nullptr, 0);
    a.spec_out = reinterpret_cast<float2 *>(d_spectra);
    a.spec_stride = stride;
    HIP_TRY(ro::launch_stft(h->bins, format, a, (hipStream_t)stream));
    return RO_OK;
}
// ... 639 lines not shown
```

### radio-observer_amd/csrc/ro_stream.cpp

```cpp
#include "ro_host.h"

using namespace ro::host;

namespace {

Batch *acquire_batch(ro_stft *h)
{
    if (!h->batch_pool.empty()) {
        Batch *b = h->batch_pool.back();
        h->batch_pool.pop_back();
        return b;
    }
    Batch *b = new (std::nothrow) Batch();
    if (!b) return nullptr;
    b->capacity_rows = h->batch_rows;
    const size_t cap = (size_t)b->capacity_rows;
    if ((!h->sink && b->data.alloc(cap * h->out_cols) != hipSuccess) ||
        b->records.alloc(cap) != hipSuccess ||
        (h->extra_count > 0 && b->extra.alloc(cap * h->extra_count) != hipSuccess) ||
        (h->cfg.tile_ln && (b->ln.alloc(cap * h->out_cols) != hipSuccess || b->minmax.alloc(cap * 2) != hipSuccess)) ||
        hipEventCreateWithFlags(&b->done, hipEventDisableTiming) != hipSuccess ||
        hipEventCreate(&b->k0) != hipSuccess || hipEventCreate(&b->k1) != hipSuccess) {
        destroy_batch(b);
        return nullptr;
    }
    return b;
}

void release_batch(ro_stft *h, Batch *b)
{
    b->consumed = 0;
    b->rows = 0;
    b->pending = false;
    h->batch_pool.push_back(b);
}

size_t stage_sample_bytes(const ro_stft *h) { return h->stage_fmt == RO_IQ_I16 ? 4 : h->stage_fmt == RO_IQ_F64 ? 16 : 8; }
size_t slot_sample_bytes(const ro_stft *h) { return h->f64reg ? 16 : 8; }

int ensure_stream_slots(ro_stft *h)
{
    if (h->slots_ready) return RO_OK;
    HIP_TRY(hipSetDevice(h->device));
    const size_t in_samples = (size_t)(h->batch_rows - 1) * h->hop + h->bins;
    hipError_t e = hipSuccess;
    auto ok = [&](hipError_t r) { if (e == hipSuccess) e = r; return e == hipSuccess; };
    ok(hipStreamCreateWithFlags(&h->s_in, hipStreamNonBlocking)) && ok(hipStreamCreateWithFlags(&h->s_out, hipStreamNonBlocking));
    for (auto &sl : h->slot) {
        ok(sl.d_iq.alloc(in_samples * slot_sample_bytes(h))) &&
            ok(sl.d_rows.alloc((size_t)h->batch_rows * h->bins)) &&
            ok(sl.d_records.alloc((size_t)h->batch_rows)) &&
            ok(sl.h_in.alloc(in_samples * slot_sample_bytes(h))) &&
            ok(hipEventCreateWithFlags(&sl.uploaded, hipEventDisableTiming)) &&
            ok(hipEventCreateWithFlags(&sl.computed, hipEventDisableTiming)) &&
            ok(hipEventCreateWithFlags(&sl.drained, hipEventDisableTiming));
        if (h->cfg.tile_cols > 0)
            ok(sl.d_tile.alloc((size_t)h->batch_rows * h->cfg.tile_cols));
        if (h->extra_count > 0)
            ok(sl.d_extra.alloc((size_t)h->batch_rows * h->extra_count));
        if (h->tile_win_count > 0)
            ok(sl.d_image.alloc((size_t)h->batch_rows * h->tile_win_total));
        if (h->cfg.tile_ln)
            ok(sl.d_ln.alloc((size_t)h->batch_rows * h->cfg.tile_cols)) && ok(sl.d_minmax.alloc((size_t)h->batch_rows * 2));
    }
    if (e != hipSuccess) {
        free_stream_slots(h);
        return fail(RO_ERR_HIP, "allocating the streaming buffers failed: %s", hipGetErrorString(e));
    }
    h->slots_ready = true;
    return RO_OK;
}

int await_batch(ro_stft *h, Batch *b)
{
    if (!b->pending) return RO_OK;
    HIP_TRY(hipEventSynchronize(b->done));
    b->pending = false;
    float ms = 0.f;
    h->timing.batches += 1;
    h->timing.batch_rows += b->rows;
    if (b->timed && hipEventElapsedTime(&ms, b->k0, b->k1) == hipSuccess) {
        h->stat_kernel_ms += ms;
        h->timed_batches += 1;
        h->timed_rows += b->rows;
        h->batch_ms_sum += ms;
        h->last_batch_ms = ms;
        h->timing.batch_gpu_ms_max = std::max(h->timing.batch_gpu_ms_max, (double)ms);
    } else if (!b->timed) {
        h->stat_kernel_ms += h->last_batch_ms;
    }
    return RO_OK;
}

int run_stream_batch(ro_stft *h, int64_t rows)
{
    if (rows <= 0) return RO_OK;
    HIP_TRY(hipSetDevice(h->device));
    const size_t sb = stage_sample_bytes(h);
    const int64_t need = (rows - 1) * (int64_t)h->hop + h->bins;
    if ((int64_t)h->staged_have < need) return fail(RO_ERR_STATE, "internal: %lld samples staged, %lld needed",
                                                    (long long)h->staged_have, (long long)need);
    if (h->sink && h->rows_ready + rows > h->sink_cap)
        return fail(RO_ERR_STATE, "row sink full: %lld rows wait to be fetched in a ring of %lld slots", (long long)h->rows_ready,
                    (long long)h->sink_cap);
    ro_stft::Slot &sl = h->slot[h->batch_seq % RO_STREAM_SLOTS];
    constexpr size_t MAX_IN_FLIGHT = 4;
    if (h->ready.size() >= MAX_IN_FLIGHT) {
        const int wrc = await_batch(h, h->ready[h->ready.size() - MAX_IN_FLIGHT]);
        if (wrc != RO_OK) return wrc;
    }
    Batch *b = acquire_batch(h);
    if (!b) return fail(RO_ERR_NOMEM, "out of pinned host memory for a row batch");
    int rc = RO_OK;
    auto step = [&](hipError_t e, const char *what) {
        if (rc == RO_OK && e != hipSuccess) rc = fail(RO_ERR_HIP, "%s failed: %s", what, hipGetErrorString(e));
        return rc == RO_OK;
    };
    const bool small = (size_t)h->batch_rows * h->out_cols * sizeof(float) <= ((size_t)4 << 20);
    bool graphed = RO_STREAM_GRAPH && small && h->sink && !h->cfg.tile_ln && (!h->f64 || h->f64reg) && !h->czt && !h->four &&
                   rows == h->batch_rows && sl.uses > 0;
    ro_scan_record_t *g_recs = h->cfg.enable_scan ? sl.d_records : nullptr;
    ro_scan_record_t *g_ext = h->extra_count > 0 ? sl.d_extra : nullptr;
    const size_t ext_bytes = (size_t)rows * (size_t)h->extra_count * sizeof(ro_scan_record_t);
    if (graphed && (!sl.gexec || sl.graph_fmt != h->stage_fmt)) {
        if (sl.gexec) { (void)hipGraphExecDestroy(sl.gexec); sl.gexec = nullptr; }
        if (!sl.gstream) step(hipStreamCreateWithFlags(&sl.gstream, hipStreamNonBlocking), "hipStreamCreateWithFlags");
        if (h->f64reg) step(ro::f64reg_prepare(h->bins, h->stage_fmt), "f64reg_prepare");
        hipGraph_t g = nullptr;
        if (rc == RO_OK && step(hipStreamBeginCapture(sl.gstream, hipStreamCaptureModeThreadLocal), "hipStreamBeginCapture")) {
            step(hipMemcpyAsync(sl.d_iq, sl.h_in, (size_t)need * sb, hipMemcpyHostToDevice, sl.gstream), "upload");
            if (rc == RO_OK) rc = launch_transform(h, sl.d_iq, h->stage_fmt, 0, rows, sl.d_rows, h->bins, sl.gstream, sl.d_tile, g_recs, sl.d_ln);
            if (rc == RO_OK) rc = launch_tile_and_scan(h, sl.d_rows, h->bins, rows, sl.d_tile, g_recs, sl.gstream, sl.d_ln, sl.d_minmax, g_ext);
            const hipError_t ce = hipStreamEndCapture(sl.gstream, &g);
            if (rc == RO_OK) step(ce, "hipStreamEndCapture");
            if (rc == RO_OK) step(hipGraphInstantiate(&sl.gexec, g, nullptr, nullptr, 0), "hipGraphInstantiate");
            if (g) (void)hipGraphDestroy(g);
        }
        if (rc != RO_OK) {
            (void)hipGetLastError();
            sl.gexec = nullptr;
            h->graph_refused = true;
            rc = RO_OK;
        }
        sl.graph_fmt = h->stage_fmt;
    }
    graphed = graphed && sl.gexec && !h->graph_refused;
    if (graphed != sl.on_gstream && sl.uses > 0) {
        if (sl.on_gstream) step(hipStreamSynchronize(sl.gstream), "hipStreamSynchronize");
        else step(hipStreamSynchronize(h->s_out), "hipStreamSynchronize");
    }
    sl.on_gstream = graphed;
    sl.uses += 1;
    if (graphed) {
        hipStream_t gs = sl.gstream;
        const int every = h->diag_time_every > 0 ? h->diag_time_every : RO_GRAPH_TIME_EVERY;
        b->timed = h->graph_batches++ % every == 0;
        if (b->timed) step(hipEventRecord(b->k0, gs), "hipEventRecord");
        if (h->diag_direct) {
            step(hipMemcpyAsync(sl.d_iq, sl.h_in, (size_t)need * sb, hipMemcpyHostToDevice, gs), "upload");
            if (rc == RO_OK) rc = launch_transform(h, sl.d_iq, h->stage_fmt, 0, rows, sl.d_rows, h->bins, gs, sl.d_tile, g_recs, sl.d_ln);
            if (rc == RO_OK) rc = launch_tile_and_scan(h, sl.d_rows, h->bins, rows, sl.d_tile, g_recs, gs, sl.d_ln, sl.d_minmax, g_ext);
        } else {
            step(hipGraphLaunch(sl.gexec, gs), "hipGraphLaunch");
        }
        if (b->timed) step(hipEventRecord(b->k1, gs), "hipEventRecord");
        if (!h->diag_done_only) {
            step(hipEventRecord(sl.uploaded, gs), "hipEventRecord");
            sl.staging_free = sl.uploaded;
        } else {
            sl.staging_free = b->done;
        }
        if (rc == RO_OK) {
            const float *src = h->cfg.tile_cols > 0 ? sl.d_tile : sl.d_rows;
            const size_t w = (size_t)h->out_cols * sizeof(float);
            const int64_t s0 = (h->sink_first + h->rows_emitted) % h->sink_cap;
            const int64_t n0 = std::min<int64_t>(rows, h->sink_cap - s0);
            step(hipMemcpy2DAsync(h->sink + s0 * h->sink_stride, (size_t)h->sink_stride * sizeof(float), src, w, w, (size_t)n0,
                                  hipMemcpyDeviceToHost, gs), "download");
            if (n0 < rows)
                step(hipMemcpy2DAsync(h->sink, (size_t)h->sink_stride * sizeof(float), src + (size_t)n0 * h->out_cols, w, w,
                                      (size_t)(rows - n0), hipMemcpyDeviceToHost, gs), "download");
            if (h->cfg.enable_scan)
                step(hipMemcpyAsync(b->records, sl.d_records, (size_t)rows * sizeof(ro_scan_record_t), hipMemcpyDeviceToHost, gs),
                     "download");
            if (g_ext) step(hipMemcpyAsync(b->extra, sl.d_extra, ext_bytes, hipMemcpyDeviceToHost, gs), "download");
        }
        step(hipEventRecord(b->done, gs), "hipEventRecord");
    } else {
    step(hipStreamWaitEvent(h->s_in, sl.computed, 0), "hipStreamWaitEvent") &&
        step(hipMemcpyAsync(sl.d_iq, sl.h_in, (size_t)need * sb, hipMemcpyHostToDevice, h->s_in), "upload") &&
        step(hipEventRecord(sl.uploaded, h->s_in), "hipEventRecord");
    sl.staging_free = sl.uploaded;
    b->timed = true;
    step(hipStreamWaitEvent(h->stream, sl.uploaded, 0), "hipStreamWaitEvent") &&
        step(hipStreamWaitEvent(h->stream, sl.drained, 0), "hipStreamWaitEvent") &&
        step(hipEventRecord(b->k0, h->stream), "hipEventRecord");
    if (rc == RO_OK) {
        ro_scan_record_t *recs = h->cfg.enable_scan ? sl.d_records : nullptr;
        const ro::CutArgs cut = make_cut_args(h->tile_win, h->tile_win_count, sl.d_image, h->tile_win_total);
        rc = launch_transform(h, sl.d_iq, h->stage_fmt, 0, rows, sl.d_rows, h->bins, h->stream, sl.d_tile, recs, sl.d_ln);
        if (rc == RO_OK)
            rc = launch_tile_and_scan(h, sl.d_rows, h->bins, rows, sl.d_tile, recs, h->stream, sl.d_ln, sl.d_minmax, g_ext,
                                      h->tile_win_count > 0 ? &cut : nullptr);
    }
    step(hipEventRecord(b->k1, h->stream), "hipEventRecord") && step(hipEventRecord(sl.computed, h->stream), "hipEventRecord");
    step(hipStreamWaitEvent(h->s_out, sl.computed, 0), "hipStreamWaitEvent");
    if (rc == RO_OK) {
        const float *src = h->tile_win_count > 0 ? sl.d_image : h->cfg.tile_cols > 0 ? sl.d_tile : sl.d_rows;
        if (h->sink) {
            const size_t w = (size_t)h->out_cols * sizeof(float);
            const int64_t s0 = (h->sink_first + h->rows_emitted) % h->sink_cap;
            const int64_t n0 = std::min<int64_t>(rows, h->sink_cap - s0);
            step(hipMemcpy2DAsync(h->sink + s0 * h->sink_stride, (size_t)h->sink_stride * sizeof(float), src, w, w, (size_t)n0,
                                  hipMemcpyDeviceToHost, h->s_out), "download");
            if (n0 < rows)
                step(hipMemcpy2DAsync(h->sink, (size_t)h->sink_stride * sizeof(float), src + (size_t)n0 * h->out_cols, w, w,
                                      (size_t)(rows - n0), hipMemcpyDeviceToHost, h->s_out), "download");
        } else {
            step(hipMemcpyAsync(b->data, src, (size_t)rows * h->out_cols * sizeof(float), hipMemcpyDeviceToHost, h->s_out),
                 "download");
        }
        if (h->cfg.enable_scan)
            step(hipMemcpyAsync(b->records, sl.d_records, (size_t)rows * sizeof(ro_scan_record_t), hipMemcpyDeviceToHost,
                                h->s_out), "download");
        if (g_ext) step(hipMemcpyAsync(b->extra, sl.d_extra, ext_bytes, hipMemcpyDeviceToHost, h->s_out), "download");
        if (h->cfg.tile_ln) {
            step(hipMemcpyAsync(b->ln, sl.d_ln, (size_t)rows * h->out_cols * sizeof(float), hipMemcpyDeviceToHost, h->s_out),
                 "download");
            step(hipMemcpyAsync(b->minmax, sl.d_minmax, (size_t)rows * 2 * sizeof(float), hipMemcpyDeviceToHost, h->s_out),
                 "download");
        }
    }
    step(hipEventRecord(sl.drained, h->s_out), "hipEventRecord") && step(hipEventRecord(b->done, h->s_out), "hipEventRecord");
    }
    if (rc != RO_OK) {
        (void)hipStreamSynchronize(h->s_in);
        (void)hipStreamSynchronize(h->stream);
        (void)hipStreamSynchronize(h->s_out);
        for (ro_stft::Slot &o : h->slot)
            if (o.gstream) (void)hipStreamSynchronize(o.gstream);
        release_batch(h, b);
        return rc;
    }
    b->first_row = h->rows_emitted;
    b->rows = rows;
    b->pending = true;
    h->batch_seq += 1;
    h->stat_launches += 1;
    h->stat_rows += rows;

    const int64_t consumed = rows * (int64_t)h->hop;
    h->stream_sample0 += consumed;
    h->rows_emitted += rows;
    h->rows_ready += rows;
    h->ready.push_back(b);
    ro_stft::Slot &nx = h->slot[h->batch_seq % RO_STREAM_SLOTS];
    const hipError_t we = hipEventSynchronize(nx.staging_free ? nx.staging_free : nx.uploaded);
    const size_t left = h->staged_have - (size_t)consumed;
    std::memcpy(nx.h_in, static_cast<const char *>(sl.h_in) + (size_t)consumed * sb, left * sb);
    h->staged_have = left;
    if (we != hipSuccess) return fail(RO_ERR_HIP, "hipEventSynchronize failed: %s", hipGetErrorString(we));
    return RO_OK;
}

int64_t staged_complete_rows(const ro_stft *h)
{
    const int64_t have = (int64_t)h->staged_have;
    if (have < h->bins) return 0;
    return (have - h->bins) / h->hop + 1;
}

}

namespace ro {
namespace host {

void destroy_batch(Batch *b)
{
    if (b->done) (void)hipEventDestroy(b->done);
    if (b->k0) (void)hipEventDestroy(b->k0);
    if (b->k1) (void)hipEventDestroy(b->k1);
    delete b;
}

void free_stream_slots(ro_stft *h)
{
    for (auto &sl : h->slot) {
        if (sl.uploaded) (void)hipEventDestroy(sl.uploaded);
        if (sl.computed) (void)hipEventDestroy(sl.computed);
        if (sl.drained) (void)hipEventDestroy(sl.drained);
        if (sl.gexec) (void)hipGraphExecDestroy(sl.gexec);
        if (sl.gstream) (void)hipStreamDestroy(sl.gstream);
        sl = ro_stft::Slot();
    }
    if (h->s_in) (void)hipStreamDestroy(h->s_in);
    if (h->s_out) (void)hipStreamDestroy(h->s_out);
    h->s_in = h->s_out = nullptr;
    h->slots_ready = false;
}

}
}

extern "C" int ro_stft_push(ro_stft_t *h, const void *iq, int format, int64_t samples, int64_t *rows_ready)
{
    if (!h) return fail(RO_ERR_INVALID, "null handle");
    if (samples < 0 || (samples > 0 && !iq)) return fail(RO_ERR_INVALID, "bad sample buffer");
    if (format != RO_IQ_F32 && format != RO_IQ_I16 && format != RO_IQ_F64)
        return fail(RO_ERR_INVALID, "unknown sample format %d", format);
    const double t0 = now_ms();
    int rc = ensure_stream_slots(h);
    if (rc != RO_OK) return rc;

    const bool in_i16 = format == RO_IQ_I16;
    const int want_fmt = in_i16 ? RO_IQ_I16 : (format == RO_IQ_F64 && h->f64reg) ? RO_IQ_F64 : RO_IQ_F32;
    const size_t cap = (size_t)(h->batch_rows - 1) * h->hop + h->bins;
    auto rank_of = [](int f) { return f == RO_IQ_I16 ? 0 : f == RO_IQ_F32 ? 1 : 2; };
    if (!h->stage_fmt_set) {
        h->stage_fmt = want_fmt;
        h->stage_fmt_set = true;
    } else if (rank_of(want_fmt) > rank_of(h->stage_fmt)) {
        char *base = static_cast<char *>(h->slot[h->batch_seq % RO_STREAM_SLOTS].h_in);
        const size_t n = h->staged_have * 2;
        if (h->stage_fmt == RO_IQ_I16 && want_fmt == RO_IQ_F32) {
            const int16_t *src = reinterpret_cast<const int16_t *>(base);
            float *dst = reinterpret_cast<float *>(base);
            for (size_t i = n; i-- > 0;) dst[i] = (float)src[i];
        } else if (h->stage_fmt == RO_IQ_I16) {
            const int16_t *src = reinterpret_cast<const int16_t *>(base);
            double *dst = reinterpret_cast<double *>(base);
            for (size_t i = n; i-- > 0;) dst[i] = (double)src[i];
        } else {
            const float *src = reinterpret_cast<const float *>(base);
            double *dst = reinterpret_cast<double *>(base);
            for (size_t i = n; i-- > 0;) dst[i] = (double)src[i];
        }
        h->stage_fmt = want_fmt;
    }
    if (h->sink) {
        const size_t spent = (size_t)h->batch_rows * h->hop;
        size_t have = h->staged_have;
        int64_t batches = 0;
        for (int64_t left = samples; left > 0;) {
            const int64_t take = std::min<int64_t>(left, (int64_t)(cap - have));
            have += (size_t)take;
            left -= take;
            if (have == cap) { ++batches; have -= spent; }
        }
        if (h->rows_ready + batches * (int64_t)h->batch_rows > h->sink_cap)
            return fail(RO_ERR_STATE, "row sink full: this push would complete %lld rows with %lld waiting to be fetched in a "
                                      "ring of %lld slots; nothing was consumed -- fetch, then push the same samples again",
                        (long long)(batches * h->batch_rows), (long long)h->rows_ready, (long long)h->sink_cap);
    }
    const size_t sb = stage_sample_bytes(h);
    const size_t isb = format == RO_IQ_F64 ? 16 : format == RO_IQ_F32 ? 8 : 4;
    const char *in = static_cast<const char *>(iq);
    h->stat_samples += samples;
    for (int64_t left = samples; left > 0;) {
        char *dstb = static_cast<char *>(h->slot[h->batch_seq % RO_STREAM_SLOTS].h_in) + h->staged_have * sb;
        const int64_t take = std::min<int64_t>(left, (int64_t)(cap - h->staged_have));
        if (h->stage_fmt == RO_IQ_I16) {
            std::memcpy(dstb, in, (size_t)take * 4);
        } else if (h->stage_fmt == RO_IQ_F64) {
            double *dst = reinterpret_cast<double *>(dstb);
            if (format == RO_IQ_F64) {
                std::memcpy(dst, in, (size_t)take * 2 * sizeof(double));
            } else if (in_i16) {
                const int16_t *src = reinterpret_cast<const int16_t *>(in);
                for (int64_t i = 0; i < take * 2; ++i) dst[i] = (double)src[i];
            } else {
                const float *src = reinterpret_cast<const float *>(in);
                for (int64_t i = 0; i < take * 2; ++i) dst[i] = (double)src[i];
            }
        } else {
            float *dst = reinterpret_cast<float *>(dstb);
            if (format == RO_IQ_F32) {
                std::memcpy(dst, in, (size_t)take * 2 * sizeof(float));
            } else if (in_i16) {
                const int16_t *src = reinterpret_cast<const int16_t *>(in);
                for (int64_t i = 0; i < take * 2; ++i) dst[i] = (float)src[i];
            } else {
                const double *src = reinterpret_cast<const double *>(in);
                size_t nt_from = (size_t)8 << 20;
#ifdef RO_DIAG_KNOBS
                if (const char *e = getenv("RO_STAGE_NT_BYTES")) nt_from = (size_t)atoll(e);
#endif
                const bool past_caches = cap * sb > nt_from;
                for (int64_t at = 0; at < take * 2; at += (int64_t)1 << 30) {
                    const int n = (int)std::min<int64_t>(take * 2 - at, (int64_t)1 << 30);
                    if (past_caches) ro::narrowToFloatStream(src + at, dst + at, n);
                    else ro::narrowToFloat(src + at, dst + at, n);
                }
            }
        }
        h->staged_have += (size_t)take;
        in += (size_t)take * isb;
        left -= take;
        if (h->staged_have == cap) {
            rc = run_stream_batch(h, h->batch_rows);
            if (rc != RO_OK) return rc;
        }
    }
    if (rows_ready) *rows_ready = h->rows_ready;
    const double dt = now_ms() - t0;
    h->timing.push_calls += 1;
    h->push_ms_sum += dt;
    h->timing.push_ms_max = std::max(h->timing.push_ms_max, dt);
    return RO_OK;
}

extern "C" int ro_stft_flush(ro_stft_t *h, int64_t *rows_ready)
{
    if (!h) return fail(RO_ERR_INVALID, "null handle");
    while (h->slots_ready) {
        const int64_t n = std::min<int64_t>(staged_complete_rows(h), h->batch_rows);
        if (n <= 0) break;
        int rc = run_stream_batch(h, n);
        if (rc != RO_OK) return rc;
    }
    if (rows_ready) *rows_ready = h->rows_ready;
    return RO_OK;
}

static int fetch_rows(ro_stft_t *h, int64_t max_rows, int first_col, int cols, float *rows_out, ro_scan_record_t *records_out,
                      ro_scan_record_t *extra_out, int64_t *first_row_index, int64_t *rows_got)
{
    if (!h || !rows_got) return fail(RO_ERR_INVALID, "null argument");
    if (extra_out && h->extra_count == 0)
        return fail(RO_ERR_STATE, "extra records requested but no extra band sets are set (ro_stft_set_extra_bands)");
    if (max_rows < 0) return fail(RO_ERR_INVALID, "negative max_rows");
    if (rows_out && (first_col < h->out_first || cols <= 0 || first_col + cols > h->out_first + h->out_cols))
        return fail(RO_ERR_INVALID, "columns [%d,+%d) outside [%d,+%d) -- what this handle brings to the host%s",
                    first_col, cols, h->out_first, h->out_cols,
                    h->tile_win_count > 0 ? " (image columns of its tile windows)" : h->cfg.tile_cols > 0 ? " (the configured tile)" : "");
    if (records_out && !h->cfg.enable_scan) return fail(RO_ERR_STATE, "scan records requested but scan is off");
    if (rows_out && h->sink) return fail(RO_ERR_STATE, "this handle's rows go to its row sink (ro_stft_set_row_sink): pass rows_out = NULL");
    const double t0 = now_ms();
    int64_t got = 0;
    if (first_row_index) *first_row_index = h->rows_emitted;
    if (first_row_index && !h->ready.empty())
        *first_row_index = h->ready.front()->first_row + h->ready.front()->consumed;
    while (got < max_rows && !h->ready.empty()) {
        Batch *b = h->ready.front();
        { const int rc = await_batch(h, b); if (rc != RO_OK) return rc; }
        const int64_t take = std::min(max_rows - got, b->rows - b->consumed);
        for (int64_t r = 0; r < take; ++r) {
            if (rows_out) {
                const float *src = b->data + (size_t)(b->consumed + r) * h->out_cols + (first_col - h->out_first);
                std::memcpy(rows_out + (size_t)(got + r) * cols, src, sizeof(float) * cols);
            }
            if (records_out) records_out[got + r] = b->records[(size_t)(b->consumed + r)];
        }
        if (extra_out)
            std::memcpy(extra_out + (size_t)got * h->extra_count, b->extra + (size_t)b->consumed * h->extra_count,
                        sizeof(ro_scan_record_t) * (size_t)take * h->extra_count);
        b->consumed += take;
        got += take;
        if (b->consumed == b->rows) {
            h->ready.pop_front();
            release_batch(h, b);
        }
    }
    h->rows_ready -= got;
    *rows_got = got;
    const double dt = now_ms() - t0;
    h->timing.fetch_calls += 1;
    h->fetch_ms_sum += dt;
    h->timing.fetch_ms_max = std::max(h->timing.fetch_ms_max, dt);
    return RO_OK;
}

extern "C" int ro_stft_fetch(ro_stft_t *h, int64_t max_rows, int first_col, int cols, float *rows_out,
                             ro_scan_record_t *records_out, int64_t *first_row_index, int64_t *rows_got)
{
    return fetch_rows(h, max_rows, first_col, cols, rows_out, records_out, nullptr, first_row_index, rows_got);
}

extern "C" int ro_stft_fetch_sets(ro_stft_t *h, int64_t max_rows, int first_col, int cols, float *rows_out,
                                  ro_scan_record_t *records_out, ro_scan_record_t *extra_out, int64_t *first_row_index,
                                  int64_t *rows_got)
{
    return fetch_rows(h, max_rows, first_col, cols, rows_out, records_out, extra_out, first_row_index, rows_got);
}

extern "C" int ro_stft_set_extra_bands(ro_stft_t *h, const ro_bands_t *sets, int count)
{
    if (!h) return fail(RO_ERR_INVALID, "null handle");
    if (count < 0 || count > RO_MAX_EXTRA_BANDS)
        return fail(RO_ERR_INVALID, "%d extra band sets: a handle takes 0 ... %d", count, RO_MAX_EXTRA_BANDS);
    if (count > 0 && !sets) return fail(RO_ERR_INVALID, "null band sets");
    if (count > 0 && !h->cfg.enable_scan)
        return fail(RO_ERR_STATE, "extra band sets need a primary set (enable_scan / ro_stft_set_bands)");
    if (!h->ready.empty() || h->staged_have > 0)
        return fail(RO_ERR_STATE, "the extra band sets can only change on an idle stream (after create or ro_stft_reset)");
    for (int i = 0; i < count; ++i)
        if (const int rc = check_bands(h, sets[i])) {
            const std::string why = last_error_text();
            return fail(rc, "extra band set %d: %s", i, why.c_str());
        }
    HIP_TRY(hipSetDevice(h->device));
    if (h->s_in) HIP_TRY(hipStreamSynchronize(h->s_in));
    if (h->stream) HIP_TRY(hipStreamSynchronize(h->stream));
    if (h->s_out) HIP_TRY(hipStreamSynchronize(h->s_out));
    for (auto &sl : h->slot) {
        if (sl.gstream) HIP_TRY(hipStreamSynchronize(sl.gstream));
        if (sl.gexec) { (void)hipGraphExecDestroy(sl.gexec); sl.gexec = nullptr; }
        sl.d_extra.reset();
    }
    while (!h->batch_pool.empty()) { destroy_batch(h->batch_pool.back()); h->batch_pool.pop_back(); }
    h->extra_count = 0;
    if (h->slots_ready && count > 0)
        for (auto &sl : h->slot)
            HIP_TRY(sl.d_extra.alloc((size_t)h->batch_rows * count));
    for (int i = 0; i < count; ++i) h->extra[i] = sets[i];
    h->extra_count = count;
    return RO_OK;
}

extern "C" int ro_stft_set_tile_windows(ro_stft_t *h, const ro_band_window_t *windows, int count)
{
    if (!h) return fail(RO_ERR_INVALID, "null handle");
    if (h->cfg.tile_cols > 0 || h->cfg.tile_ln)
        return fail(RO_ERR_UNSUPPORTED, "tile windows are for handles created without a tile (tile_cols = %d, tile_ln = %d)",
                    h->cfg.tile_cols, h->cfg.tile_ln);
    int64_t total = 0;
    if (count != 0) {
        const int rc = tile_windows_check("ro_stft_set_tile_windows", h->bins, windows, count, &total);
        if (rc != RO_OK) return rc;
    }
    if (h->sink) return fail(RO_ERR_STATE, "this handle's rows go to its row sink (ro_stft_set_row_sink): remove it first");
    if (!h->ready.empty() || h->staged_have > 0)
        return fail(RO_ERR_STATE, "the tile windows can only change on an idle stream (after create or ro_stft_reset)");
    HIP_TRY(hipSetDevice(h->device));
    if (h->s_in) HIP_TRY(hipStreamSynchronize(h->s_in));
    if (h->stream) HIP_TRY(hipStreamSynchronize(h->stream));
    if (h->s_out) HIP_TRY(hipStreamSynchronize(h->s_out));
    for (auto &sl : h->slot) {
        if (sl.gstream) HIP_TRY(hipStreamSynchronize(sl.gstream));
        sl.d_image.reset();
    }
    while (!h->batch_pool.empty()) { destroy_batch(h->batch_pool.back()); h->batch_pool.pop_back(); }
    h->tile_win_count = 0;
    h->tile_win_total = 0;
    h->out_first = 0;
    h->out_cols = h->bins;
    if (count == 0) return RO_OK;
    if (h->slots_ready)
        for (auto &sl : h->slot)
            HIP_TRY(sl.d_image.alloc((size_t)h->batch_rows * (size_t)total));
    for (int i = 0; i < count; ++i) h->tile_win[i] = windows[i];
    h->tile_win_count = count;
    h->tile_win_total = (int)total;
    h->out_cols = (int)total;
    return RO_OK;
}

extern "C" int ro_stft_tile_windows(const ro_stft_t *h, ro_band_window_t *out)
{
    if (!h) return fail(RO_ERR_INVALID, "null handle");
    if (out)
        for (int i = 0; i < h->tile_win_count; ++i) out[i] = h->tile_win[i];
    return h->tile_win_count;
}

extern "C" int ro_stft_rows_complete(ro_stft_t *h, int64_t *rows)
{
    if (!h || !rows) return fail(RO_ERR_INVALID, "null argument");
    int64_t n = 0;
    for (Batch *b : h->ready) {
        if (b->pending) {
            const hipError_t e = hipEventQuery(b->done);
            if (e == hipErrorNotReady) break;
            if (e != hipSuccess) return fail(RO_ERR_HIP, "hipEventQuery failed: %s", hipGetErrorString(e));
            const int rc = await_batch(h, b);
            if (rc != RO_OK) return rc;
        }
        n += b->rows - b->consumed;
    }
    *rows = n;
    return RO_OK;
}

extern "C" int ro_stft_fetch_ln(ro_stft_t *h, int64_t max_rows, float *tile_out, float *ln_out, float *minmax_out,
                                ro_scan_record_t *records_out, int64_t *first_row_index, int64_t *rows_got)
{
    if (!h || !rows_got) return fail(RO_ERR_INVALID, "null argument");
    if (!h->cfg.tile_ln) return fail(RO_ERR_STATE, "this handle was not created with tile_ln");
    if (max_rows < 0) return fail(RO_ERR_INVALID, "negative max_rows");
    if (records_out && !h->cfg.enable_scan) return fail(RO_ERR_STATE, "scan records requested but scan is off");
    const double t0 = now_ms();
    int64_t got = 0;
    if (first_row_index) *first_row_index = h->rows_emitted;
    if (first_row_index && !h->ready.empty())
        *first_row_index = h->ready.front()->first_row + h->ready.front()->consumed;
    const size_t w = (size_t)h->out_cols;
    while (got < max_rows && !h->ready.empty()) {
        Batch *b = h->ready.front();
        { const int rc = await_batch(h, b); if (rc != RO_OK) return rc; }
        const int64_t take = std::min(max_rows - got, b->rows - b->consumed);
        const size_t at = (size_t)b->consumed;
        if (tile_out) std::memcpy(tile_out + (size_t)got * w, b->data + at * w, sizeof(float) * w * (size_t)take);
        if (ln_out) std::memcpy(ln_out + (size_t)got * w, b->ln + at * w, sizeof(float) * w * (size_t)take);
        if (minmax_out) std::memcpy(minmax_out + (size_t)got * 2, b->minmax + at * 2, sizeof(float) * 2 * (size_t)take);
        if (records_out) std::memcpy(records_out + got, b->records + at, sizeof(ro_scan_record_t) * (size_t)take);
        b->consumed += take;
        got += take;
        if (b->consumed == b->rows) {
            h->ready.pop_front();
            release_batch(h, b);
        }
    }
    h->rows_ready -= got;
    *rows_got = got;
    const double dt = now_ms() - t0;
    h->timing.fetch_calls += 1;
    h->fetch_ms_sum += dt;
    h->timing.fetch_ms_max = std::max(h->timing.fetch_ms_max, dt);
    return RO_OK;
}

extern "C" int ro_stft_set_row_sink(ro_stft_t *h, float *base, int64_t row_stride, int64_t capacity_rows, int64_t first_slot)
{
    if (!h) return fail(RO_ERR_INVALID, "null handle");
    if (!h->ready.empty() || h->staged_have > 0)
        return fail(RO_ERR_STATE, "the row sink can only change on an idle stream (after create or ro_stft_reset)");
    if (h->cfg.tile_ln) return fail(RO_ERR_UNSUPPORTED, "a tile_ln handle hands its rows out through ro_stft_fetch_ln");
    if (h->tile_win_count > 0)
        return fail(RO_ERR_STATE, "a handle with tile windows hands its image out through ro_stft_fetch: remove the windows first "
                                  "(ro_stft_set_tile_windows with count = 0)");
    HIP_TRY(hipSetDevice(h->device));
    while (!h->batch_pool.empty()) { destroy_batch(h->batch_pool.back()); h->batch_pool.pop_back(); }
    h->sink = nullptr;
    if (!base) return RO_OK;
    const int cols = h->cfg.tile_cols > 0 ? h->cfg.tile_cols : h->bins;
    if (row_stride < cols || capacity_rows < 2 * (int64_t)h->batch_rows || first_slot < 0 || first_slot >= capacity_rows)
        return fail(RO_ERR_INVALID, "row sink: stride %lld (rows are %d wide), %lld slots (two batches of %d rows at least), "
                                    "first slot %lld", (long long)row_stride, cols, (long long)capacity_rows, h->batch_rows,
                    (long long)first_slot);
    {
        const size_t bytes = ((size_t)(capacity_rows - 1) * (size_t)row_stride + (size_t)cols) * sizeof(float);
        if (ro_pinned_check(base, bytes) != 1)
            return fail(RO_ERR_INVALID, "row sink: [%p, +%zu bytes) is not page-locked host memory of this process's HIP runtime "
                                        "(use ro_pinned_alloc)", (const void *)base, bytes);
    }
    h->sink = base;
    h->sink_stride = row_stride;
    h->sink_cap = capacity_rows;
    h->sink_first = first_slot;
    return RO_OK;
}

extern "C" int ro_stft_reset(ro_stft_t *h)
{
    if (!h) return fail(RO_ERR_INVALID, "null handle");
    if (h->s_in) (void)hipStreamSynchronize(h->s_in);
    if (h->stream) (void)hipStreamSynchronize(h->stream);
    if (h->s_out) (void)hipStreamSynchronize(h->s_out);
    for (auto &sl : h->slot)
        if (sl.gstream) (void)hipStreamSynchronize(sl.gstream);
    h->staged_have = 0;
    h->stage_fmt_set = false;
    while (!h->ready.empty()) {
        release_batch(h, h->ready.front());
        h->ready.pop_front();
    }
    h->stream_sample0 = 0;
    h->rows_emitted = 0;
    h->rows_ready = 0;
    return RO_OK;
}
```

### radio-observer_amd/host/HipWaterfallBackend.cpp

```cpp
#if defined(__SSE2__)
#include <emmintrin.h>
#endif
#include "HipWaterfallBackend.h"
#include "../csrc/ro_narrow.h"

#include <sys/time.h>

#include <algorithm>
#include <cerrno>
#include <climits>
#include <cstdio>
#include <cmath>
#include <cstdlib>
#include <cstring>

namespace ro {

static int wrapIndex(int value, int size)
{
    while (value < 0) value += size;
    return value % size;
}

int Recorder::getSampleRate() const { return backend_->streamInfo().sampleRate; }
// ... 77 lines not shown

void WaterfallBase::pushRaw(const Complex *data, size_t n)
{
    if (!cfg_.keep_raw || rawBuffer_.getCapacity() == 0) return;
    rawBuffer_.pushRun((int)n, [&](float *rows, int count, int done) {
        narrowToFloatStream(&data[done].real, rows, 2 * count);
    });
}

void WaterfallBase::finishStream()
{
    for (Recorder *r : recorders_) r->stop();
}

void WaterfallBase::processRow(const float *row, const ro_scan_record_t *scan, DataInfo info, int rawMark)
{
    processRow(row, scan, nullptr, 0, info, rawMark);
}

void WaterfallBase::processRow(const float *row, const ro_scan_record_t *scan, const ro_scan_record_t *extra, int extraCount,
                               DataInfo info, int rawMark)
{
    {
        std::lock_guard<std::mutex> g(bufferMutex_);
        float *dst = buffer_.push();
        if (row) std::memcpy(dst, row, sizeof(float) * (size_t)bins_);
        rawHandles_[buffer_.mark()] = RawDataHandle(rawMark, info.timeOffset);
    }
    if (scan) currentScan_[0] = *scan;
    for (int s = 0; extra && s < extraCount && 1 + s < MAX_SCAN_SETS; ++s) currentScan_[1 + s] = extra[s];
    rowsDelivered_++;
    if (keepLog_) rowLog_.push_back(RowInfo{info.offset, info.timeOffset, rawMark});
    for (Recorder *r : recorders_) r->update();
}

bool parseWaterfallKeys(const std::map<std::string, std::string> &keys, WaterfallConfig *cfg, std::string *err)
{
    WaterfallConfig c = *cfg;
    std::string why;
    auto asInt = [&](const char *key, int *out) {
        auto it = keys.find(key);
        if (it == keys.end()) return true;
        const char *s = it->second.c_str();
        char *end = nullptr;
        errno = 0;
        const long v = std::strtol(s, &end, 10);
        if (end == s || *end != '\0' || errno != 0 || v < INT_MIN || v > INT_MAX) {
            why = std::string("waterfall: \"") + key + "\" must be an integer, got \"" + it->second + "\"";
            return false;
        }
        *out = (int)v;
        return true;
    };
    auto asDouble = [&](const char *key, double *out) {
        auto it = keys.find(key);
        if (it == keys.end()) return true;
        const char *s = it->second.c_str();
        char *end = nullptr;
        errno = 0;
        const double v = std::strtod(s, &end);
        if (end == s || *end != '\0' || errno != 0) {
            why = std::string("waterfall: \"") + key + "\" must be a number, got \"" + it->second + "\"";
            return false;
        }
        *out = v;
        return true;
    };
    auto asString = [&](const char *key, std::string *out) {
        auto it = keys.find(key);
        if (it != keys.end()) *out = it->second;
    };
    bool ok = asInt("bins", &c.bins) && asInt("overlap", &c.overlap) && asInt("buffer_chunk_size", &c.buffer_chunk_size) &&
              asDouble("iq_gain", &c.iq_gain) && asInt("iq_phase_shift", &c.iq_phase_shift);
    asString("origin", &c.origin);
    asString("metadata_path", &c.metadata_path);
    auto it = keys.find("precision");
    if (ok && it != keys.end()) {
        if (it->second == "f32") c.precision = RO_PRECISION_F32;
        else if (it->second == "f64") c.precision = RO_PRECISION_F64;
        else {
            why = "waterfall: unknown \"precision\" \"" + it->second + "\" (expected \"f32\" or \"f64\")";
            ok = false;
        }
    }
    if (!ok) {
        if (err) *err = why;
        return false;
    }
    *cfg = c;
    if (err) err->clear();
    return true;
}

HipWaterfallBackend::HipWaterfallBackend(const WaterfallConfig &cfg) : WaterfallBase(cfg)
{
    buffer_.setStorage(pinnedAlloc, pinnedFree, &cfg_.device);
}

HipWaterfallBackend::~HipWaterfallBackend()
{
    if (stft_) ro_stft_destroy(stft_);
}

void HipWaterfallBackend::startStream(StreamInfo info)
{
    Backend::startStream(info);
    samplesIn_ = 0;
    inMark_ = 0;
    nextStampRow_ = 0;
    rowTimes_.clear();

    if (stft_) { ro_stft_destroy(stft_); stft_ = nullptr; }
    ro_stft_config_t c;
    std::memset(&c, 0, sizeof(c));
    scanEnabled_ = beginStream(info, &c.bands);
    if (!streamError_.empty()) {
        lastError_ = streamError_;
        std::fprintf(stderr, "HipWaterfallBackend: %s\n", lastError_.c_str());
        return;
    }
    c.struct_size = sizeof(c);
    c.bins = bins_;
    c.overlap = overlap_;
    c.sample_rate = info.sampleRate;
    c.window_kind = RO_WINDOW_NUTTALL;
    c.iq_gain = cfg_.iq_gain;
    c.iq_phase_shift = cfg_.iq_phase_shift;
    c.device = cfg_.device;
    c.precision = cfg_.precision;
    batchRows_ = cfg_.max_batch_rows;
    if (batchRows_ <= 0) {
        const int64_t one_second = (int64_t)std::ceil((double)fftSampleRate_);
        const int64_t ring = buffer_.getCapacity() / 8;
        const int64_t raw = cfg_.keep_raw ? (int64_t)rawCapacity_ / hop_ / 4 : one_second;
        batchRows_ = (int)std::max<int64_t>(1, std::min<int64_t>(std::min(one_second, ring), std::min<int64_t>(raw, 4096)));
    }
    if (cfg_.keep_raw && (int64_t)batchRows_ * hop_ + bins_ > rawCapacity_)
        std::fprintf(stderr, "HipWaterfallBackend: batch of %d rows (%lld samples) exceeds the raw ring (%d samples): "
                             "raw captures of events will hold newer samples than their rows\n",
                     batchRows_, (long long)batchRows_ * hop_ + bins_, rawCapacity_);
    c.max_batch_rows = batchRows_;
    auto lagFits = [&](int64_t batches) {
        return batches * (int64_t)batchRows_ <= buffer_.getCapacity() / 4 &&
               (!cfg_.keep_raw || batches * (int64_t)batchRows_ * hop_ + bins_ <= rawCapacity_ / 2);
    };
    maxOutstanding_ = lagFits(4) ? 3 : lagFits(3) ? 2 : 1;
    c.enable_scan = scanEnabled_ ? 1 : 0;
    if (ro_stft_create(&c, &stft_) != RO_OK) {
        lastError_ = ro_last_error();
        std::fprintf(stderr, "HipWaterfallBackend: %s\n", lastError_.c_str());
        stft_ = nullptr;
        return;
    }
    if (!extraBands_.empty() && ro_stft_set_extra_bands(stft_, extraBands_.data(), (int)extraBands_.size()) != RO_OK) {
        lastError_ = ro_last_error();
        std::fprintf(stderr, "HipWaterfallBackend: %s\n", lastError_.c_str());
        ro_stft_destroy(stft_);
        stft_ = nullptr;
        return;
    }
    rowSink_ = buffer_.storageIsCustom() &&
               ro_stft_set_row_sink(stft_, buffer_.data(), bins_, buffer_.getCapacity(), buffer_.mark()) == RO_OK;
}

void HipWaterfallBackend::stampRowStarts(int64_t takeBegin, int64_t takeEnd, const WFTime &t)
{
    while (nextStampRow_ * (int64_t)hop_ < takeEnd) {
        const int64_t s = nextStampRow_ * (int64_t)hop_;
        if (s >= takeBegin) rowTimes_.push_back(t.addSamples((SampleCount)(s - takeBegin), info_.sampleRate));
        nextStampRow_++;
    }
}

void HipWaterfallBackend::process(const std::vector<Complex> &data, DataInfo info)
{
    if (!stft_ || data.empty()) return;
    {
        int64_t size = (int64_t)data.size();
        int64_t pos = samplesIn_;
        WFTime timeOffset = info.timeOffset;
        while (size >= bins_ - inMark_) {
            const int count = bins_ - inMark_;
            stampRowStarts(pos, pos + count, timeOffset);
            inMark_ = overlap_;
            size -= count;
            pos += count;
            timeOffset = timeOffset.addSamples((SampleCount)count, info_.sampleRate);
        }
        if (size > 0) {
            stampRowStarts(pos, pos + size, timeOffset);
            inMark_ += (int)size;
        }
        samplesIn_ += (int64_t)data.size();
    }
    const size_t piece = std::max<size_t>((size_t)hop_, (size_t)(buffer_.getCapacity() / 4) * (size_t)hop_);
    for (size_t at = 0; at < data.size(); at += piece) {
        const Complex *src = data.data() + at;
        const size_t n = std::min(piece, data.size() - at);
        int64_t ready = 0;
        if (rowSink_) {
            const int64_t upTo = samplesIn_ - (int64_t)data.size() + (int64_t)(at + n);
            const int64_t complete = upTo >= bins_ ? (upTo - bins_) / hop_ + 1 : 0;
            int64_t ahead = complete - rowsDelivered_;
            if (ahead > buffer_.getCapacity() / 2) {
                drain(false, true);
                ahead = complete - rowsDelivered_;
            }
            if (ahead > 0) {
                std::lock_guard<std::mutex> g(bufferMutex_);
                buffer_.markAhead((int)std::min<int64_t>(ahead, buffer_.getCapacity()));
            }
        }
        pushRaw(src, n);
        const int rc = ro_stft_push(stft_, src, RO_IQ_F64, (int64_t)n, &ready);
        if (rc != RO_OK) {
            lastError_ = ro_last_error();
            std::fprintf(stderr, "HipWaterfallBackend: %s\n", lastError_.c_str());
            return;
        }
        drain(false);
    }
}

void HipWaterfallBackend::endStream()
{
    Backend::endStream();
    if (stft_) drain(true);
    finishStream();
}

void HipWaterfallBackend::drain(bool flush, bool wait)
{
    int64_t ready = 0;
    if (flush && ro_stft_flush(stft_, &ready) != RO_OK) {
        drain(false, true);
        if (ro_stft_flush(stft_, &ready) != RO_OK) {
            lastError_ = ro_last_error();
            return;
        }
    }
    const int64_t CH = 64;
    if (!rowSink_) fetchRows_.resize((size_t)CH * bins_);
    fetchRecs_.resize((size_t)CH);
    const int nExtra = scanEnabled_ ? (int)extraBands_.size() : 0;
    fetchExtra_.resize((size_t)CH * (size_t)nExtra);
    int64_t budget = -1;
    if (!flush && !wait) {
        if (ro_stft_rows_complete(stft_, &budget) != RO_OK) {
            lastError_ = ro_last_error();
            return;
        }
    }
    for (;;) {
        int64_t first = 0, got = 0;
        if (budget == 0) {
            int64_t launched = 0;
            if (ro_stft_stats(stft_, nullptr, &launched, nullptr, nullptr) != RO_OK) break;
            if (launched - rowsFetched_ <= (int64_t)maxOutstanding_ * batchRows_) break;
            budget = launched - rowsFetched_ - (int64_t)maxOutstanding_ * batchRows_;
        }
        const int64_t want = budget < 0 ? CH : std::min<int64_t>(CH, budget);
        const int frc = nExtra > 0
            ? ro_stft_fetch_sets(stft_, want, 0, bins_, rowSink_ ? nullptr : fetchRows_.data(), fetchRecs_.data(),
                                 fetchExtra_.data(), &first, &got)
            : ro_stft_fetch(stft_, want, 0, bins_, rowSink_ ? nullptr : fetchRows_.data(),
                            scanEnabled_ ? fetchRecs_.data() : nullptr, &first, &got);
        if (frc != RO_OK) {
            lastError_ = ro_last_error();
            return;
        }
        if (got == 0) break;
        if (budget > 0) budget -= got;
        rowsFetched_ += got;
        for (int64_t i = 0; i < got; ++i) {
            const int64_t r = first + i;
            DataInfo di;
            di.offset = (SampleCount)r;
            di.timeOffset = rowTimes_.empty() ? WFTime() : rowTimes_.front();
            if (!rowTimes_.empty()) rowTimes_.pop_front();
            const int64_t s = (overlap_ > 0 ? (r + 1) : r) * (int64_t)hop_;
            const int rawMark = (int)((s + 1) % rawCapacity_);
            processRow(rowSink_ ? nullptr : &fetchRows_[(size_t)i * bins_], scanEnabled_ ? &fetchRecs_[(size_t)i] : nullptr,
                       nExtra > 0 ? &fetchExtra_[(size_t)i * (size_t)nExtra] : nullptr, nExtra, di, rawMark);
        }
    }
}

}
```

### radio-observer_amd/host/HipWaterfallBackend.h

```cpp
#pragma once

#include <deque>
#include <map>
#include <memory>
#include <mutex>
#include <string>
#include <vector>

#include "../../include/ro_stft.h"
#include "Backend.h"
#include "CsvLog.h"
#include "RingBuffer.h"

namespace ro {

struct RawDataHandle {
    int    mark = 0;
    WFTime time;
    RawDataHandle() {}
    RawDataHandle(int m, WFTime t) : mark(m), time(t) {}
};

class WaterfallBase;

// ... 29 lines not shown
    int                         scanSlot_ = 0;
    WaterfallBase              *backend_;
    RingBuffer2D<float>        *buffer_ = nullptr;
    RingBuffer2D<float>        *rawBuffer_ = nullptr;
    std::mutex                 *bufferMutex_ = nullptr;
    std::vector<RawDataHandle> *rawHandles_ = nullptr;
};

struct WaterfallConfig {
    int         bins = 32768;
    int         overlap = 0;
    std::string origin = "debug";
    std::string metadata_path = ".";
    int         buffer_chunk_size = 1024 * 1024;
    double      iq_gain = 0.0;
    int         iq_phase_shift = 0;
    int         device = 0;
    int         max_batch_rows = 0;
    bool        keep_raw = true;
    int         precision = RO_PRECISION_F32;
};

bool parseWaterfallKeys(const std::map<std::string, std::string> &keys, WaterfallConfig *cfg, std::string *err);

class WaterfallBase {
public:
    explicit WaterfallBase(const WaterfallConfig &cfg);
    virtual ~WaterfallBase() {}

    int   getBins() const { return bins_; }
    float getFFTSampleRate() const { return fftSampleRate_; }
    SampleType getGain() const { return cfg_.iq_gain; }
    StreamInfo streamInfo() const { return info_; }
    float binToFrequency(int bin) const { return ro_bin_to_frequency(bins_, info_.sampleRate, bin); }
    float binToFrequency() const { return binToFrequency(1) - binToFrequency(0); }
    int   frequencyToBin(float f) const { return ro_frequency_to_bin(bins_, info_.sampleRate, f); }
    double fftSamplesToTime(int samples) const { return (double)samples / (double)fftSampleRate_; }
    int   timeToFFTSamples(double t) const { return ro_time_to_fft_samples(t, fftSampleRate_); }
    int   fftSamplesToRaw(int sampleCount) const
    {
        return (int)(((double)sampleCount / (double)fftSampleRate_) * (double)info_.sampleRate);
    }
    std::string getOrigin() const { return cfg_.origin; }
    const WaterfallConfig &config() const { return cfg_; }

    void addRecorder(Recorder *recorder);

    CsvLog *getMetadataFile();
    struct Noise { float noise = 0, peakFrequency = 0, magnitude = 0; };
    void publishNoise(float n, float peakFq, float mag) { lastNoise_ = Noise{n, peakFq, mag}; }
    const Noise &lastNoise() const { return lastNoise_; }
    WFTime now() const;
    void setClock(WFTime fixed) { fixedClock_ = fixed; useFixedClock_ = true; }

    static constexpr int MAX_SCAN_SETS = 1 + RO_MAX_EXTRA_BANDS;
    const ro_scan_record_t &currentScan() const { return currentScan_[0]; }
    const ro_scan_record_t &currentScan(int slot) const { return currentScan_[slot >= 0 && slot < MAX_SCAN_SETS ? slot : 0]; }
    const std::vector<ro_bands_t> &extraBands() const { return extraBands_; }
    const std::string &streamError() const { return streamError_; }
    bool  scanEnabled() const { return scanEnabled_; }
    int64_t currentRowIndex() const { return rowsDelivered_ - 1; }

    RingBuffer2D<float> &buffer() { return buffer_; }
    RingBuffer2D<float> &rawBuffer() { return rawBuffer_; }
    const std::vector<RawDataHandle> &rawHandles() const { return rawHandles_; }
    int64_t rowsDelivered() const { return rowsDelivered_; }
    int rawCapacity() const { return rawCapacity_; }
    struct RowInfo { uint64_t offset; WFTime time; int rawMark; };
    const std::vector<RowInfo> &rowLog() const { return rowLog_; }
    void keepRowLog(bool on) { keepLog_ = on; }

protected:
    bool beginStream(const StreamInfo &info, ro_bands_t *bands);
    void finishStream();
    virtual void processRow(const float *row, const ro_scan_record_t *scan, DataInfo info, int rawMark);
    virtual void processRow(const float *row, const ro_scan_record_t *scan, const ro_scan_record_t *extra, int extraCount,
                            DataInfo info, int rawMark);

    WaterfallConfig cfg_;
    StreamInfo info_;
    int   bins_, overlap_, hop_;
    float fftSampleRate_ = 0.f;
    bool  scanEnabled_ = false;

    void pushRaw(const Complex *data, size_t n);

    std::unique_ptr<CsvLog>    metadataFile_;
    Noise  lastNoise_;
    WFTime fixedClock_;
    bool   useFixedClock_ = false;
    RingBuffer2D<float>        buffer_;
    std::mutex                 bufferMutex_;
    RingBuffer2D<float>        rawBuffer_;
    std::vector<RawDataHandle> rawHandles_;
    std::vector<Recorder *>    recorders_;
    int     rawCapacity_ = 1;
    int     maxOutstanding_ = 1;
    int64_t rowsDelivered_ = 0;
    int64_t rowsFetched_ = 0;
    ro_scan_record_t currentScan_[MAX_SCAN_SETS] = {};
    std::vector<ro_bands_t> extraBands_;
    std::string streamError_;
    std::vector<RowInfo> rowLog_;
    bool keepLog_ = false;
};

class ManualWaterfall : public WaterfallBase {
public:
    explicit ManualWaterfall(const WaterfallConfig &cfg) : WaterfallBase(cfg) {}
    bool startStream(const StreamInfo &info)
    {
        ro_bands_t b;
        scanEnabled_ = beginStream(info, &b);
        return streamError_.empty();
    }
    void pushSamples(const Complex *data, size_t n) { pushRaw(data, n); }
    void pushRow(const float *row, const ro_scan_record_t *scan, WFTime time, int rawMark)
    {
        DataInfo di;
        di.offset = (SampleCount)rowsDelivered_;
        di.timeOffset = time;
        processRow(row, scan, di, rawMark);
    }
    void pushRow(const float *row, const ro_scan_record_t *scan, const ro_scan_record_t *extra, int extraCount, WFTime time,
                 int rawMark)
    {
        DataInfo di;
        di.offset = (SampleCount)rowsDelivered_;
        di.timeOffset = time;
        processRow(row, scan, extra, extraCount, di, rawMark);
    }
    void endStream() { finishStream(); }
};

class HipWaterfallBackend : public Backend, public WaterfallBase {
public:
    explicit HipWaterfallBackend(const WaterfallConfig &cfg);
    ~HipWaterfallBackend() override;

    void startStream(StreamInfo info) override;
    void process(const std::vector<Complex> &data, DataInfo info) override;
    void endStream() override;
    const std::string &lastError() const { return lastError_; }
    int batchRows() const { return batchRows_; }
    bool rowsByDma() const { return rowSink_; }
    bool timing(ro_stft_timing_t *out, bool reset) const { return stft_ && ro_stft_timing(stft_, out, reset ? 1 : 0) == RO_OK; }

private:
    void drain(bool flush, bool wait = false);
    void stampRowStarts(int64_t takeBegin, int64_t takeEnd, const WFTime &t);

    ro_stft_t *stft_ = nullptr;
    int batchRows_ = 0;
    bool rowSink_ = false;
    std::string lastError_;

    int64_t samplesIn_ = 0;
    int     inMark_ = 0;
    int64_t nextStampRow_ = 0;
    std::deque<WFTime> rowTimes_;
    std::vector<float> fetchRows_;
    std::vector<ro_scan_record_t> fetchRecs_;
    std::vector<ro_scan_record_t> fetchExtra_;
};

}
```

Baseline: 16.51 million rows/s.

## Coalesce staged streaming batches into larger adaptive kernel launches

Adds a stream plan that sizes streaming slots to hold up to a coalesce cap of rows (default 256 rows or 64 MiB), and launches several whole batches in one run when enough samples are staged. Launches are held back while the earlier batch is still running, so more rows accumulate per launch, and fetch paths flush any held-back work. This is meant to cut per-launch and graph overhead, at the cost of larger buffers, higher latency, and more complex sink/backpressure logic in the host backend. It also replaces a stream sync with a per-slot event sync.

```diff
diff --git a/include/ro_stft.h b/include/ro_stft.h
--- a/include/ro_stft.h
+++ b/include/ro_stft.h
@@ -481,6 +481,25 @@
 int ro_stft_stats(const ro_stft_t *h, int64_t *samples_in, int64_t *rows_out,
                   int64_t *launches, double *kernel_ms_total);
 
+typedef struct ro_stream_plan {
+    int64_t coalesce_rows;
+    int64_t slot_samples;
+    int64_t slot_in_bytes;
+    int64_t slot_row_floats;
+    int64_t reserved[4];
+} ro_stream_plan_t;
+int ro_stream_plan(int bins, int overlap, int64_t batch_rows, int64_t coalesce_rows, int64_t sink_capacity_rows,
+                   int sample_bytes, ro_stream_plan_t *out);
+int ro_stft_set_coalesce_rows(ro_stft_t *h, int64_t rows);
+typedef struct ro_stft_coalesce {
+    int64_t coalesce_rows;
+    int64_t coalesced_launches;
+    int64_t largest_batch_rows;
+    int64_t graphed_batches;
+    int64_t reserved[4];
+} ro_stft_coalesce_t;
+int ro_stft_coalesce(ro_stft_t *h, ro_stft_coalesce_t *out, int reset);
+
 #ifdef __cplusplus
 }
 #endif
diff --git a/radio-observer_amd/__init__.py b/radio-observer_amd/__init__.py
--- a/radio-observer_amd/__init__.py
+++ b/radio-observer_amd/__init__.py
@@ -15,7 +15,7 @@
     PERIODIC_SUMMARY_DTYPE, RO_MAX_PERIODIC, RO_PERIODIC_WRITTEN, RO_PERIODIC_LOST, RO_PERIODIC_NO_ROOM,
     snapshot_levels_host, periodic_levels_host, LEVEL_RANGE_DTYPE, RO_LEVEL_BLOCK,
     png_bytes, levels_png_host, levels_png_deflate_host, periodic_level_dir, RO_PNG_ALIGN,
-    resize_shape, resize_plan, levels_resize_host, RESIZE_INFO_DTYPE,
+    resize_shape, resize_plan, levels_resize_host, RESIZE_INFO_DTYPE, stream_plan,
     RO_WINDOW_NUTTALL, RO_WINDOW_HANN, RO_WINDOW_CUSTOM, RO_IQ_F32, RO_IQ_I16, RO_IQ_F64,
     RO_PRECISION_F32, RO_PRECISION_F64,
 )
diff --git a/radio-observer_amd/build.py b/radio-observer_amd/build.py
--- a/radio-observer_amd/build.py
+++ b/radio-observer_amd/build.py
@@ -7,7 +7,7 @@
 LIB = os.path.join(HERE, "libro_stft.so")
 SOURCES = ["ro_kernels.hip", "ro_stft32k.hip", "ro_fourstep.hip", "ro_f64reg.hip", "ro_band.hip", "ro_band_f64.hip", "ro_band_windows.hip", "ro_band_windows_f64.hip", "ro_scan_sets.hip", "ro_cut_windows.hip", "ro_events.hip", "ro_snapshots.hip", "ro_raw.hip", "ro_units.hip", "ro_periodic.hip", "ro_levels.hip", "ro_png.hip", "ro_png_deflate.hip", "ro_resize.hip", "ro_stft_capi.cpp", "ro_abi_helpers.cpp",
            "ro_exchange.cpp", "ro_stream.cpp", "ro_czt.cpp", "ro_snapshots.cpp", "ro_raw.cpp", "ro_units.cpp", "ro_periodic.cpp", "ro_levels.cpp", "ro_png.cpp", "ro_png_deflate.cpp", "ro_resize.cpp"]
-HEADERS = ["ro_kernels.h", "ro_band.h", "ro_band_f64.h", "ro_band_windows.h", "ro_events.h", "ro_snapshots.h", "ro_raw.h", "ro_units.h", "ro_periodic.h", "ro_levels.h", "ro_png.h", "ro_png_deflate.h", "ro_resize.h", "ro_png_crc_device.h", "ro_pack_plan.h", "ro_host.h", "ro_owned.h", "ro_fft_device.h", "ro_fft_planar.h", "ro_k32_lds.h", "ro_device_util.h", "ro_f64_device.h", "ro_narrow.h", os.path.join("..", "..", "include", "ro_stft.h")]
+HEADERS = ["ro_kernels.h", "ro_band.h", "ro_band_f64.h", "ro_band_windows.h", "ro_events.h", "ro_snapshots.h", "ro_raw.h", "ro_units.h", "ro_periodic.h", "ro_levels.h", "ro_png.h", "ro_png_deflate.h", "ro_resize.h", "ro_png_crc_device.h", "ro_pack_plan.h", "ro_host.h", "ro_owned.h", "ro_fft_device.h", "ro_fft_planar.h", "ro_k32_lds.h", "ro_device_util.h", "ro_f64_device.h", "ro_narrow.h", "ro_stream_plan.h", os.path.join("..", "..", "include", "ro_stft.h")]
 
 HIPCC_FLAGS = ["-O3", "--offload-arch=gfx950", "-std=c++17", "-fno-slp-vectorize", "-fPIC", "-shared",
                "-Wall", "-Wno-unused-function", "-Wno-inline-asm"]
diff --git a/radio-observer_amd/capi.py b/radio-observer_amd/capi.py
--- a/radio-observer_amd/capi.py
+++ b/radio-observer_amd/capi.py
@@ -114,6 +114,16 @@
 LEVEL_RANGE_DTYPE = np.dtype([("ln_min", np.float32), ("ln_max", np.float32)])
 RESIZE_INFO_DTYPE = np.dtype([("jobs", np.int64), ("h_items", np.int64), ("v_items", np.int64), ("mid_bytes", np.int64),
                               ("plan_bytes", np.int64), ("reserved", np.int64, (3,))])
+
+
+class StreamPlan(C.Structure):
+    _fields_ = [("coalesce_rows", C.c_int64), ("slot_samples", C.c_int64), ("slot_in_bytes", C.c_int64),
+                ("slot_row_floats", C.c_int64), ("reserved", C.c_int64 * 4)]
+
+
+class Coalesce(C.Structure):
+    _fields_ = [("coalesce_rows", C.c_int64), ("coalesced_launches", C.c_int64), ("largest_batch_rows", C.c_int64),
+                ("graphed_batches", C.c_int64), ("reserved", C.c_int64 * 4)]
 
 
 class Config(C.Structure):
@@ -278,6 +288,9 @@
     "ro_stft_timing": (C.c_int, [C.c_void_p, C.c_void_p, C.c_int]),
     "ro_stft_stats": (C.c_int, [C.c_void_p, C.POINTER(C.c_int64), C.POINTER(C.c_int64),
                                 C.POINTER(C.c_int64), C.POINTER(C.c_double)]),
+    "ro_stream_plan": (C.c_int, [C.c_int, C.c_int, C.c_int64, C.c_int64, C.c_int64, C.c_int, C.c_void_p]),
+    "ro_stft_set_coalesce_rows": (C.c_int, [C.c_void_p, C.c_int64]),
+    "ro_stft_coalesce": (C.c_int, [C.c_void_p, C.c_void_p, C.c_int]),
 }
 
 _lib = None
@@ -773,6 +786,12 @@
     _check(library().ro_levels_resize_host(p(info), p(plan), p(levels) if levels.size else None, levels.size,
                                            p(out) if out_levels_bytes > 0 else None, out_levels_bytes))
     return out[:out_levels_bytes]
+
+
+def stream_plan(bins, overlap, batch_rows, coalesce_rows=0, sink_capacity_rows=0, sample_bytes=8):
+    p = StreamPlan()
+    _check(library().ro_stream_plan(bins, overlap, batch_rows, coalesce_rows, sink_capacity_rows, sample_bytes, C.byref(p)))
+    return {k: getattr(p, k) for k, _ in StreamPlan._fields_ if k != "reserved"}
 
 
 def device_count():
@@ -1167,6 +1186,14 @@
         _check(library().ro_stft_timing(self._h, C.byref(t), 1 if reset else 0))
         return {k: getattr(t, k) for k, _ in Timing._fields_}
 
+    def set_coalesce_rows(self, rows):
+        _check(library().ro_stft_set_coalesce_rows(self._h, rows))
+
+    def coalesce(self, reset=False):
+        c = Coalesce()
+        _check(library().ro_stft_coalesce(self._h, C.byref(c), 1 if reset else 0))
+        return {k: getattr(c, k) for k, _ in Coalesce._fields_ if k != "reserved"}
+
     def rows_complete(self):
         n = C.c_int64()
         _check(library().ro_stft_rows_complete(self._h, C.byref(n)))
diff --git a/radio-observer_amd/csrc/ro_host.h b/radio-observer_amd/csrc/ro_host.h
--- a/radio-observer_amd/csrc/ro_host.h
+++ b/radio-observer_amd/csrc/ro_host.h
@@ -33,6 +33,7 @@
 #include "ro_resize.h"
 #include "ro_narrow.h"
 #include "ro_owned.h"
+#include "ro_stream_plan.h"
 
 #if defined(RO_DIAG) && !defined(RO_DIAG_KNOBS)
 #define RO_DIAG_KNOBS 1
@@ -133,6 +134,11 @@
     int        tile_win_count = 0, tile_win_total = 0;
 
     int batch_rows = 0;
+    int64_t coalesce_req = 0;
+    int64_t coalesce_rows = 0;
+    int64_t slot_rows = 0;
+    int64_t coalesced_launches = 0, largest_batch = 0, graphed_launches = 0;
+    int64_t last_launch_rows = 0;
     int stage_fmt = RO_IQ_F32;
     bool stage_fmt_set = false;
     size_t  staged_have = 0;
@@ -357,6 +363,7 @@
 
 void destroy_batch(Batch *b);
 void free_stream_slots(ro_stft *h);
-
-}
-}
+int apply_coalesce_rows(ro_stft *h);
+
+}
+}
diff --git a/radio-observer_amd/csrc/ro_stft_capi.cpp b/radio-observer_amd/csrc/ro_stft_capi.cpp
--- a/radio-observer_amd/csrc/ro_stft_capi.cpp
+++ b/radio-observer_amd/csrc/ro_stft_capi.cpp
@@ -686,6 +686,7 @@
     h->out_cols = cfg->tile_cols > 0 ? cfg->tile_cols : h->bins;
     h->batch_rows = cfg->max_batch_rows > 0 ? cfg->max_batch_rows
                                             : std::max(1, (64 << 20) / (h->bins * 4));
+    if (const int rc = apply_coalesce_rows(h)) { ro_stft_destroy(h); return rc; }
 #ifdef RO_DIAG_KNOBS
     if (const char *e = getenv("RO_GRAPH_TIME_EVERY")) h->diag_time_every = atoi(e);
     if (const char *e = getenv("RO_GRAPH_TWO_EVENTS")) h->diag_done_only = atoi(e) == 0;
diff --git a/radio-observer_amd/csrc/ro_stream.cpp b/radio-observer_amd/csrc/ro_stream.cpp
--- a/radio-observer_amd/csrc/ro_stream.cpp
+++ b/radio-observer_amd/csrc/ro_stream.cpp
@@ -13,7 +13,7 @@
     }
     Batch *b = new (std::nothrow) Batch();
     if (!b) return nullptr;
-    b->capacity_rows = h->batch_rows;
+    b->capacity_rows = h->slot_rows;
     const size_t cap = (size_t)b->capacity_rows;
     if ((!h->sink && b->data.alloc(cap * h->out_cols) != hipSuccess) ||
         b->records.alloc(cap) != hipSuccess ||
@@ -42,31 +42,35 @@
 {
     if (h->slots_ready) return RO_OK;
     HIP_TRY(hipSetDevice(h->device));
-    const size_t in_samples = (size_t)(h->batch_rows - 1) * h->hop + h->bins;
+    ro_stream_plan_t plan;
+    if (const char *why = ro::stream_plan(h->bins, h->overlap, h->batch_rows, h->coalesce_rows, 0, (int)slot_sample_bytes(h), &plan))
+        return fail(RO_ERR_INVALID, "streaming buffers: %s", why);
+    const size_t slot_rows = (size_t)plan.coalesce_rows;
     hipError_t e = hipSuccess;
     auto ok = [&](hipError_t r) { if (e == hipSuccess) e = r; return e == hipSuccess; };
     ok(hipStreamCreateWithFlags(&h->s_in, hipStreamNonBlocking)) && ok(hipStreamCreateWithFlags(&h->s_out, hipStreamNonBlocking));
     for (auto &sl : h->slot) {
-        ok(sl.d_iq.alloc(in_samples * slot_sample_bytes(h))) &&
-            ok(sl.d_rows.alloc((size_t)h->batch_rows * h->bins)) &&
-            ok(sl.d_records.alloc((size_t)h->batch_rows)) &&
-            ok(sl.h_in.alloc(in_samples * slot_sample_bytes(h))) &&
+        ok(sl.d_iq.alloc((size_t)plan.slot_in_bytes)) &&
+            ok(sl.d_rows.alloc((size_t)plan.slot_row_floats)) &&
+            ok(sl.d_records.alloc(slot_rows)) &&
+            ok(sl.h_in.alloc((size_t)plan.slot_in_bytes)) &&
             ok(hipEventCreateWithFlags(&sl.uploaded, hipEventDisableTiming)) &&
             ok(hipEventCreateWithFlags(&sl.computed, hipEventDisableTiming)) &&
             ok(hipEventCreateWithFlags(&sl.drained, hipEventDisableTiming));
         if (h->cfg.tile_cols > 0)
-            ok(sl.d_tile.alloc((size_t)h->batch_rows * h->cfg.tile_cols));
+            ok(sl.d_tile.alloc(slot_rows * h->cfg.tile_cols));
         if (h->extra_count > 0)
-            ok(sl.d_extra.alloc((size_t)h->batch_rows * h->extra_count));
+            ok(sl.d_extra.alloc(slot_rows * h->extra_count));
         if (h->tile_win_count > 0)
-            ok(sl.d_image.alloc((size_t)h->batch_rows * h->tile_win_total));
+            ok(sl.d_image.alloc(slot_rows * h->tile_win_total));
         if (h->cfg.tile_ln)
-            ok(sl.d_ln.alloc((size_t)h->batch_rows * h->cfg.tile_cols)) && ok(sl.d_minmax.alloc((size_t)h->batch_rows * 2));
+            ok(sl.d_ln.alloc(slot_rows * h->cfg.tile_cols)) && ok(sl.d_minmax.alloc(slot_rows * 2));
     }
     if (e != hipSuccess) {
         free_stream_slots(h);
         return fail(RO_ERR_HIP, "allocating the streaming buffers failed: %s", hipGetErrorString(e));
     }
+    h->slot_rows = (int64_t)slot_rows;
     h->slots_ready = true;
     return RO_OK;
 }
@@ -147,7 +151,7 @@
     graphed = graphed && sl.gexec && !h->graph_refused;
     if (graphed != sl.on_gstream && sl.uses > 0) {
         if (sl.on_gstream) step(hipStreamSynchronize(sl.gstream), "hipStreamSynchronize");
-        else step(hipStreamSynchronize(h->s_out), "hipStreamSynchronize");
+        else step(hipEventSynchronize(sl.drained), "hipEventSynchronize");
     }
     sl.on_gstream = graphed;
     sl.uses += 1;
@@ -248,6 +252,10 @@
     h->batch_seq += 1;
     h->stat_launches += 1;
     h->stat_rows += rows;
+    h->coalesced_launches += rows > h->batch_rows ? 1 : 0;
+    h->largest_batch = std::max(h->largest_batch, rows);
+    h->graphed_launches += graphed ? 1 : 0;
+    h->last_launch_rows = rows;
 
     const int64_t consumed = rows * (int64_t)h->hop;
     h->stream_sample0 += consumed;
@@ -270,6 +278,28 @@
     return (have - h->bins) / h->hop + 1;
 }
 
+bool earlier_batch_done(ro_stft *h)
+{
+    if (h->ready.size() < 2) return true;
+    const Batch *b = h->ready[h->ready.size() - 2];
+    return !b->pending || hipEventQuery(b->done) != hipErrorNotReady;
+}
+
+int launch_whole_batches(ro_stft *h, bool full)
+{
+    int64_t n = staged_complete_rows(h);
+    if (n < h->batch_rows) return RO_OK;
+    if (!full && !earlier_batch_done(h)) return RO_OK;
+    if (!full && n < std::min(h->last_launch_rows, h->coalesce_rows) && !h->ready.empty() && h->ready.back()->pending &&
+        hipEventQuery(h->ready.back()->done) == hipErrorNotReady)
+        return RO_OK;
+    if (h->sink) n = std::min(n, h->sink_cap - h->rows_ready);
+    n -= n % h->batch_rows;
+    return run_stream_batch(h, std::min(n, h->coalesce_rows));
+}
+
+int launch_held_back(ro_stft *h) { return h->slots_ready ? launch_whole_batches(h, false) : RO_OK; }
+
 }
 
 namespace ro {
@@ -297,6 +327,26 @@
     if (h->s_out) (void)hipStreamDestroy(h->s_out);
     h->s_in = h->s_out = nullptr;
     h->slots_ready = false;
+    h->slot_rows = 0;
+}
+
+int apply_coalesce_rows(ro_stft *h)
+{
+    ro_stream_plan_t plan;
+    if (const char *why = ro::stream_plan(h->bins, h->overlap, h->batch_rows, h->coalesce_req, h->sink ? h->sink_cap : 0, 8, &plan))
+        return fail(RO_ERR_INVALID, "coalesce_rows: %s", why);
+    h->coalesce_rows = plan.coalesce_rows;
+    if (h->slots_ready && h->coalesce_rows > h->slot_rows) {
+        HIP_TRY(hipSetDevice(h->device));
+        if (h->s_in) HIP_TRY(hipStreamSynchronize(h->s_in));
+        if (h->stream) HIP_TRY(hipStreamSynchronize(h->stream));
+        if (h->s_out) HIP_TRY(hipStreamSynchronize(h->s_out));
+        for (auto &sl : h->slot)
+            if (sl.gstream) HIP_TRY(hipStreamSynchronize(sl.gstream));
+        while (!h->batch_pool.empty()) { destroy_batch(h->batch_pool.back()); h->batch_pool.pop_back(); }
+        free_stream_slots(h);
+    }
+    return RO_OK;
 }
 
 }
@@ -314,7 +364,7 @@
 
     const bool in_i16 = format == RO_IQ_I16;
     const int want_fmt = in_i16 ? RO_IQ_I16 : (format == RO_IQ_F64 && h->f64reg) ? RO_IQ_F64 : RO_IQ_F32;
-    const size_t cap = (size_t)(h->batch_rows - 1) * h->hop + h->bins;
+    const size_t cap = (size_t)(h->coalesce_rows - 1) * h->hop + h->bins;
     auto rank_of = [](int f) { return f == RO_IQ_I16 ? 0 : f == RO_IQ_F32 ? 1 : 2; };
     if (!h->stage_fmt_set) {
         h->stage_fmt = want_fmt;
@@ -338,15 +388,9 @@
         h->stage_fmt = want_fmt;
     }
     if (h->sink) {
-        const size_t spent = (size_t)h->batch_rows * h->hop;
-        size_t have = h->staged_have;
-        int64_t batches = 0;
-        for (int64_t left = samples; left > 0;) {
-            const int64_t take = std::min<int64_t>(left, (int64_t)(cap - have));
-            have += (size_t)take;
-            left -= take;
-            if (have == cap) { ++batches; have -= spent; }
-        }
+        const int64_t have = (int64_t)h->staged_have + samples;
+        const int64_t complete = have < h->bins ? 0 : (have - h->bins) / h->hop + 1;
+        const int64_t batches = complete / h->batch_rows;
         if (h->rows_ready + batches * (int64_t)h->batch_rows > h->sink_cap)
             return fail(RO_ERR_STATE, "row sink full: this push would complete %lld rows with %lld waiting to be fetched in a "
                                       "ring of %lld slots; nothing was consumed -- fetch, then push the same samples again",
@@ -396,10 +440,8 @@
         h->staged_have += (size_t)take;
         in += (size_t)take * isb;
         left -= take;
-        if (h->staged_have == cap) {
-            rc = run_stream_batch(h, h->batch_rows);
-            if (rc != RO_OK) return rc;
-        }
+        rc = launch_whole_batches(h, h->staged_have == cap);
+        if (rc != RO_OK) return rc;
     }
     if (rows_ready) *rows_ready = h->rows_ready;
     const double dt = now_ms() - t0;
@@ -413,7 +455,8 @@
 {
     if (!h) return fail(RO_ERR_INVALID, "null handle");
     while (h->slots_ready) {
-        const int64_t n = std::min<int64_t>(staged_complete_rows(h), h->batch_rows);
+        const int64_t staged = staged_complete_rows(h);
+        const int64_t n = staged >= 2 * (int64_t)h->batch_rows ? std::min(staged, h->coalesce_rows) : std::min<int64_t>(staged, h->batch_rows);
         if (n <= 0) break;
         int rc = run_stream_batch(h, n);
         if (rc != RO_OK) return rc;
@@ -437,10 +480,12 @@
     if (rows_out && h->sink) return fail(RO_ERR_STATE, "this handle's rows go to its row sink (ro_stft_set_row_sink): pass rows_out = NULL");
     const double t0 = now_ms();
     int64_t got = 0;
+    { const int rc = launch_held_back(h); if (rc != RO_OK) return rc; }
     if (first_row_index) *first_row_index = h->rows_emitted;
     if (first_row_index && !h->ready.empty())
         *first_row_index = h->ready.front()->first_row + h->ready.front()->consumed;
-    while (got < max_rows && !h->ready.empty()) {
+    while (got < max_rows) {
+        if (h->ready.empty() && (launch_held_back(h) != RO_OK || h->ready.empty())) break;
         Batch *b = h->ready.front();
         { const int rc = await_batch(h, b); if (rc != RO_OK) return rc; }
         const int64_t take = std::min(max_rows - got, b->rows - b->consumed);
@@ -511,7 +556,7 @@
     h->extra_count = 0;
     if (h->slots_ready && count > 0)
         for (auto &sl : h->slot)
-            HIP_TRY(sl.d_extra.alloc((size_t)h->batch_rows * count));
+            HIP_TRY(sl.d_extra.alloc((size_t)h->slot_rows * count));
     for (int i = 0; i < count; ++i) h->extra[i] = sets[i];
     h->extra_count = count;
     return RO_OK;
@@ -547,7 +592,7 @@
     if (count == 0) return RO_OK;
     if (h->slots_ready)
         for (auto &sl : h->slot)
-            HIP_TRY(sl.d_image.alloc((size_t)h->batch_rows * (size_t)total));
+            HIP_TRY(sl.d_image.alloc((size_t)h->slot_rows * (size_t)total));
     for (int i = 0; i < count; ++i) h->tile_win[i] = windows[i];
     h->tile_win_count = count;
     h->tile_win_total = (int)total;
@@ -578,7 +623,7 @@
         n += b->rows - b->consumed;
     }
     *rows = n;
-    return RO_OK;
+    return launch_held_back(h);
 }
 
 extern "C" int ro_stft_fetch_ln(ro_stft_t *h, int64_t max_rows, float *tile_out, float *ln_out, float *minmax_out,
@@ -590,11 +635,13 @@
     if (records_out && !h->cfg.enable_scan) return fail(RO_ERR_STATE, "scan records requested but scan is off");
     const double t0 = now_ms();
     int64_t got = 0;
+    { const int rc = launch_held_back(h); if (rc != RO_OK) return rc; }
     if (first_row_index) *first_row_index = h->rows_emitted;
     if (first_row_index && !h->ready.empty())
         *first_row_index = h->ready.front()->first_row + h->ready.front()->consumed;
     const size_t w = (size_t)h->out_cols;
-    while (got < max_rows && !h->ready.empty()) {
+    while (got < max_rows) {
+        if (h->ready.empty() && (launch_held_back(h) != RO_OK || h->ready.empty())) break;
         Batch *b = h->ready.front();
         { const int rc = await_batch(h, b); if (rc != RO_OK) return rc; }
         const int64_t take = std::min(max_rows - got, b->rows - b->consumed);
@@ -631,7 +678,7 @@
     HIP_TRY(hipSetDevice(h->device));
     while (!h->batch_pool.empty()) { destroy_batch(h->batch_pool.back()); h->batch_pool.pop_back(); }
     h->sink = nullptr;
-    if (!base) return RO_OK;
+    if (!base) return apply_coalesce_rows(h);
     const int cols = h->cfg.tile_cols > 0 ? h->cfg.tile_cols : h->bins;
     if (row_stride < cols || capacity_rows < 2 * (int64_t)h->batch_rows || first_slot < 0 || first_slot >= capacity_rows)
         return fail(RO_ERR_INVALID, "row sink: stride %lld (rows are %d wide), %lld slots (two batches of %d rows at least), "
@@ -647,6 +694,38 @@
     h->sink_stride = row_stride;
     h->sink_cap = capacity_rows;
     h->sink_first = first_slot;
+    return apply_coalesce_rows(h);
+}
+
+extern "C" int ro_stream_plan(int bins, int overlap, int64_t batch_rows, int64_t coalesce_rows, int64_t sink_capacity_rows,
+                              int sample_bytes, ro_stream_plan_t *out)
+{
+    if (const char *why = ro::stream_plan(bins, overlap, batch_rows, coalesce_rows, sink_capacity_rows, sample_bytes, out))
+        return fail(RO_ERR_INVALID, "ro_stream_plan: %s", why);
+    return RO_OK;
+}
+
+extern "C" int ro_stft_set_coalesce_rows(ro_stft_t *h, int64_t rows)
+{
+    if (!h) return fail(RO_ERR_INVALID, "null handle");
+    if (rows < 0) return fail(RO_ERR_INVALID, "negative coalesce_rows");
+    if (!h->ready.empty() || h->staged_have > 0)
+        return fail(RO_ERR_STATE, "the cap of coalescing can only change on an idle stream (after create or ro_stft_reset)");
+    h->coalesce_req = rows;
+    return apply_coalesce_rows(h);
+}
+
+extern "C" int ro_stft_coalesce(ro_stft_t *h, ro_stft_coalesce_t *out, int reset)
+{
+    if (!h) return fail(RO_ERR_INVALID, "null handle");
+    if (out) {
+        *out = ro_stft_coalesce_t{};
+        out->coalesce_rows = h->coalesce_rows;
+        out->coalesced_launches = h->coalesced_launches;
+        out->largest_batch_rows = h->largest_batch;
+        out->graphed_batches = h->graphed_launches;
+    }
+    if (reset) h->coalesced_launches = h->largest_batch = h->graphed_launches = 0;
     return RO_OK;
 }
 
@@ -659,6 +738,7 @@
     for (auto &sl : h->slot)
         if (sl.gstream) (void)hipStreamSynchronize(sl.gstream);
     h->staged_have = 0;
+    h->last_launch_rows = 0;
     h->stage_fmt_set = false;
     while (!h->ready.empty()) {
         release_batch(h, h->ready.front());
diff --git a/radio-observer_amd/csrc/ro_stream_plan.h b/radio-observer_amd/csrc/ro_stream_plan.h
--- /dev/null
+++ b/radio-observer_amd/csrc/ro_stream_plan.h
@@ -0,0 +1,41 @@
+#pragma once
+
+#include <cstdint>
+
+#include "../../include/ro_stft.h"
+
+namespace ro {
+
+constexpr int64_t STREAM_COALESCE_ROWS = 256;
+constexpr int64_t STREAM_COALESCE_BYTES = (int64_t)64 << 20;
+
+inline const char *stream_plan(int bins, int overlap, int64_t batch_rows, int64_t coalesce_rows, int64_t sink_capacity_rows,
+                               int sample_bytes, ro_stream_plan_t *out)
+{
+    if (!out) return "null plan";
+    if (bins < 2 || overlap < 0 || overlap >= bins) return "bins < 2 or overlap outside [0, bins)";
+    if (batch_rows < 1) return "batch_rows < 1";
+    if (coalesce_rows < 0) return "negative coalesce_rows";
+    if (sink_capacity_rows < 0) return "negative sink_capacity_rows";
+    if (sink_capacity_rows > 0 && sink_capacity_rows / 2 < batch_rows) return "a row sink shorter than two batches";
+    if (sample_bytes != 4 && sample_bytes != 8 && sample_bytes != 16) return "sample_bytes is not 4, 8 or 16";
+    int64_t cap = coalesce_rows;
+    if (cap == 0) {
+        const int64_t by_bytes = STREAM_COALESCE_BYTES / ((int64_t)bins * (int64_t)sizeof(float));
+        cap = STREAM_COALESCE_ROWS < by_bytes ? STREAM_COALESCE_ROWS : by_bytes;
+    }
+    if (sink_capacity_rows > 0 && cap > sink_capacity_rows / 2) cap = sink_capacity_rows / 2;
+    if (cap < batch_rows) cap = batch_rows;
+    cap -= cap % batch_rows;
+    const int64_t hop = bins - overlap;
+    const int64_t limit = INT64_MAX / 16;
+    if (cap > (limit - bins) / hop || cap > limit / bins) return "the slot's sizes overflow";
+    *out = ro_stream_plan_t{};
+    out->coalesce_rows = cap;
+    out->slot_samples = (cap - 1) * hop + bins;
+    out->slot_in_bytes = out->slot_samples * sample_bytes;
+    out->slot_row_floats = cap * bins;
+    return nullptr;
+}
+
+}
diff --git a/radio-observer_amd/host/HipWaterfallBackend.cpp b/radio-observer_amd/host/HipWaterfallBackend.cpp
--- a/radio-observer_amd/host/HipWaterfallBackend.cpp
+++ b/radio-observer_amd/host/HipWaterfallBackend.cpp
@@ -253,6 +253,20 @@
         stft_ = nullptr;
         return;
     }
+    const int64_t lagRows = std::min<int64_t>(buffer_.getCapacity() / 4,
+                                              cfg_.keep_raw ? ((int64_t)rawCapacity_ / 2 - bins_) / hop_ : buffer_.getCapacity() / 4);
+    ro_stream_plan_t plan;
+    std::memset(&plan, 0, sizeof plan);
+    const int64_t ringRows = buffer_.storageIsCustom() && buffer_.getCapacity() >= 2 * (int64_t)batchRows_ ? buffer_.getCapacity() : 0;
+    const bool coalesce = ro_stream_plan(bins_, overlap_, batchRows_, 0, ringRows, 8, &plan) == RO_OK &&
+                          plan.coalesce_rows > batchRows_ && plan.coalesce_rows + 2 * (int64_t)batchRows_ <= lagRows;
+    if (!coalesce && ro_stft_set_coalesce_rows(stft_, batchRows_) != RO_OK) {
+        lastError_ = ro_last_error();
+        std::fprintf(stderr, "HipWaterfallBackend: %s\n", lastError_.c_str());
+        ro_stft_destroy(stft_);
+        stft_ = nullptr;
+        return;
+    }
     if (!extraBands_.empty() && ro_stft_set_extra_bands(stft_, extraBands_.data(), (int)extraBands_.size()) != RO_OK) {
         lastError_ = ro_last_error();
         std::fprintf(stderr, "HipWaterfallBackend: %s\n", lastError_.c_str());
@@ -262,6 +276,13 @@
     }
     rowSink_ = buffer_.storageIsCustom() &&
                ro_stft_set_row_sink(stft_, buffer_.data(), bins_, buffer_.getCapacity(), buffer_.mark()) == RO_OK;
+    ro_stft_coalesce_t co;
+    std::memset(&co, 0, sizeof co);
+    outstandingRows_ = (int64_t)maxOutstanding_ * batchRows_;
+    if (coalesce && ro_stft_coalesce(stft_, &co, 0) == RO_OK && co.coalesce_rows > batchRows_) {
+        if (co.coalesce_rows + 2 * (int64_t)batchRows_ <= lagRows) outstandingRows_ = std::max(outstandingRows_, lagRows - co.coalesce_rows);
+        else (void)ro_stft_set_coalesce_rows(stft_, batchRows_);
+    }
 }
 
 void HipWaterfallBackend::stampRowStarts(int64_t takeBegin, int64_t takeEnd, const WFTime &t)
@@ -357,8 +378,8 @@
         if (budget == 0) {
             int64_t launched = 0;
             if (ro_stft_stats(stft_, nullptr, &launched, nullptr, nullptr) != RO_OK) break;
-            if (launched - rowsFetched_ <= (int64_t)maxOutstanding_ * batchRows_) break;
-            budget = launched - rowsFetched_ - (int64_t)maxOutstanding_ * batchRows_;
+            if (launched - rowsFetched_ <= outstandingRows_) break;
+            budget = launched - rowsFetched_ - outstandingRows_;
         }
         const int64_t want = budget < 0 ? CH : std::min<int64_t>(CH, budget);
         const int frc = nExtra > 0
diff --git a/radio-observer_amd/host/HipWaterfallBackend.h b/radio-observer_amd/host/HipWaterfallBackend.h
--- a/radio-observer_amd/host/HipWaterfallBackend.h
+++ b/radio-observer_amd/host/HipWaterfallBackend.h
@@ -205,6 +205,7 @@
 
     ro_stft_t *stft_ = nullptr;
     int batchRows_ = 0;
+    int64_t outstandingRows_ = 0;
     bool rowSink_ = false;
     std::string lastError_;
 
```

Measured after the change: 16.51 million rows/s, median of 2. No clear change (-0.0%).
